# showlab/VideoSwap

Hardware: NVIDIA H100
Metric: denoise-steps/sec, 16f 512^2 SD1.5 UNet3D (CFG UNet fwd + CFG combine + DDIM step) (higher is better)
Workload: dtype f16

## Files before the change

### include/videoswap_b200.h

```cpp
#ifndef VIDEOSWAP_B200_H
#define VIDEOSWAP_B200_H
#include <stddef.h>
#include <stdint.h>

#ifdef __cplusplus
extern "C" {
#endif

const char* vs_last_error(void);
int vs_version(void);

typedef struct vs_unet_config {
  int in_channels, out_channels;
  int block_out_channels[4];
  int layers_per_block;
  int num_heads;
  int cross_attention_dim;
  int norm_num_groups;
  float norm_eps;
  int use_motion_module;
  int motion_down[4];
  int motion_up[4];
  int motion_mid;
  int motion_num_heads;
  int pe_max_len;
} vs_unet_config;

typedef struct vs_unet vs_unet;

int vs_unet_create(const vs_unet_config* cfg, vs_unet** out);
void vs_unet_destroy(vs_unet* h);

int vs_unet_load_weights(vs_unet* h, void* stream, int n, const char* const* names, const void* const* d_ptrs,
                         const int64_t* numels);
int vs_unet_num_params(const vs_unet* h);
const char* vs_unet_param_name(const vs_unet* h, int i);

int vs_unet_forward(vs_unet* h, void* stream, const void* d_sample, int io_f32, int B, int F, int H, int W,
                    const float* d_timesteps, const void* d_ehs, int ehs_tokens, int ehs_layers,
                    const void* const* d_residuals, int residuals_nhwc, float residual_scale, void* d_out);
int vs_unet_forward_features(vs_unet* h, void* stream, const void* d_sample, int io_f32, int B, int F, int H, int W,
                             const float* d_timesteps, const void* d_ehs, int ehs_tokens, int ehs_layers, int up_ft_index,
                             void* d_feat);
int vs_unet_time_embedding(vs_unet* h, void* stream, const float* d_timesteps, int B, float* d_emb, float* d_proj);
size_t vs_unet_workspace_bytes(const vs_unet* h);
int vs_unet_pin_workspace(vs_unet* h, int pin);
int vs_unet_reserve_workspace(vs_unet* h, int B, int F, int H, int W);
typedef struct vs_comm vs_comm;
int vs_comm_unique_id(void* out128);
int vs_comm_create(const void* id128, int rank, int nranks, vs_comm** out);
void vs_comm_destroy(vs_comm* c);
int vs_comm_all_gather(vs_comm* c, void* stream, const void* d_send, void* d_recv, size_t bytes_per_rank);
int vs_comm_all_reduce_sum_f32(vs_comm* c, void* stream, float* d_buf, size_t n);
int vs_unet_set_frame_shard(vs_unet* h, vs_comm* frame_comm, int shard, int nshards);

typedef void (*vs_attention_hook)(void* user, int layer, int is_cross, int place, void* d_probs, int batch, int heads, int nq,
                                  int nk, void* stream);
int vs_unet_set_attention_hook(vs_unet* h, vs_attention_hook hook, void* user, int max_queries);
int vs_attention_probs(void* stream, const void* d_q, int ldq, const void* d_k, int ldk, void* d_probs, int batch, int nq, int nk,
                       int heads, int d, long long q_bstride, long long kv_bstride, int kv_div);
int vs_attention_apply_probs(void* stream, const void* d_probs, const void* d_v, int ldv, void* d_o, int ldo, int batch, int nq,
                             int nk, int heads, int d, long long kv_bstride, long long o_bstride, int kv_div);
int vs_blend_mask(void* stream, const void* const* d_maps, int n_maps, int n_prompts, int frames, int heads, int res_h, int res_w,
                  int words, const float* d_alpha, int pool, int h, int w, float threshold, int both, float* d_mask);
int vs_latent_blend(void* stream, const void* d_x_src, void* d_x_tgt, const float* d_mask, int io_f32, int channels, int frames,
                    int hw);

int vs_unet_enable_taps(vs_unet* h, int enable);
int vs_unet_num_taps(const vs_unet* h);
int vs_unet_get_tap(const vs_unet* h, int i, const char** name, const void** d_ptr, int* nimg, int* hh, int* ww, int* c);
int vs_unet_copy_tap(const vs_unet* h, void* stream, int i, void* d_dst);

int vs_cfg_ddim_step(void* stream, const void* d_eps2, const void* d_latents, int io_f32, size_t n, int cfg,
                     float guidance, float alpha_t, float alpha_prev, void* d_out);

int vs_cfg_ddim_step_dev(void* stream, const void* d_eps2, const void* d_latents, int io_f32, size_t n, int cfg,
                         float guidance, const float* d_coef, void* d_out);

int vs_cfg_ddim_rescale_step(void* stream, const void* d_eps2, const void* d_latents, const void* d_noise, int io_f32, int S,
                             size_t n_s, int cfg, float guidance, float alpha_t, float alpha_prev, float eta,
                             float guidance_rescale, void* d_out);

int vs_cfg_ddim_rescale_step_dev(void* stream, const void* d_eps2, const void* d_latents, const void* d_noise, int io_f32,
                                 int S, size_t n_s, int cfg, float guidance, const float* d_coef, void* d_out);

int vs_adapter_level(void* stream, const void* d_w0, const void* d_b0, const void* d_w1, const void* d_b1, int E, int mid,
                     int C, const float* d_point_embedding, const float* d_tracks, const int* d_point_mask, int F, int P,
                     int h, int w, float rate, int coord_fp16, float scale, float* d_ws, void* d_map);

typedef struct vs_gemm_desc {
  const void* A; int K1; int lda1;
  const void* A2; int K2; int lda2;
  const void* Bw;
  int M, N;
  int taps;
  int sub_py, sub_px;
  int nimg, H, W;
  const float* bias;
  const float* rowvec; int ldrv; int pix_per_batch; int rv_mod;
  const float* ln_stats; const float* ln_u;
  const float* ln_parts; int ln_nparts;
  float* ln_sums_out;
  const void* residual; int ldr;
  void* out; int ldc;
  int mode;
  int force_bn;
  int OH, OW;
  int stride2;
} vs_gemm_desc;
int vs_gemm_ex(void* stream, const vs_gemm_desc* desc);
int vs_pack_conv3x3(void* stream, const void* d_w, int cout, int cin, void* d_out);
int vs_pack_geglu(void* stream, const void* d_w, const void* d_b, int hidden, int K, void* d_wout, float* d_bout);
int vs_groupnorm(void* stream, const void* d_x1, int c1, const void* d_x2, int c2, int nimg, int hw, int imgs_per_set,
                 int groups, float eps, const float* d_gamma, const float* d_beta, int silu, float* d_sums, void* d_out);
int vs_groupnorm_stats(void* stream, const void* d_x1, int c1, const void* d_x2, int c2, int nimg, int hw, int imgs_per_set,
                       int groups, float* d_sums, int zero_first);
int vs_groupnorm_apply(void* stream, const void* d_x1, int c1, const void* d_x2, int c2, int nimg, int hw, int imgs_per_set,
                       int groups, const float* d_sums, float eps, const float* d_gamma, const float* d_beta, int silu,
                       int count_scale, void* d_out);
int vs_layernorm(void* stream, const void* d_x, int rows, int C, const float* d_gamma, const float* d_beta,
                 const float* d_pe, int hw, int F, void* d_out);
int vs_ln_linear(void* stream, const void* d_x, int M, int C, const void* d_w, const float* d_bias, int N,
                 const float* d_gamma, const float* d_beta, const float* d_pe, int pe_len, int hw, int frames, int mode,
                 void* d_wf, float* d_u, float* d_c, float* d_cpe, float* d_stats, void* d_out);
int vs_linear_ln_linear(void* stream, const void* d_x0, int M, int K0, const void* d_w0, const float* d_b0,
                        const void* d_residual, int C, void* d_x, const void* d_w, const float* d_bias, int N,
                        const float* d_gamma, const float* d_beta, const float* d_pe, int pe_len, int hw, int frames,
                        int mode, void* d_wf, float* d_u, float* d_c, float* d_cpe, float* d_parts, int parts_capacity,
                        void* d_out);
int vs_attention(void* stream, const void* d_q, int ldq, const void* d_k, int ldk, const void* d_v, int ldv, void* d_o,
                 int ldo, int batch, int nq, int nk, int heads, int d, long long q_bstride, long long kv_bstride,
                 long long o_bstride, int kv_div);
int vs_temporal_attention(void* stream, const void* d_qkv, void* d_o, int B, int F, int HW, int C, int heads);
int vs_conv_in(void* stream, const void* d_x, int nimg, int H, int W, int cin, const void* d_w, const float* d_bias,
               int cout, void* d_scratch, void* d_out);
int vs_upsample2x(void* stream, const void* d_x, int nimg, int H, int W, int C, void* d_out);
int vs_upsample_conv3x3(void* stream, const void* d_x, int nimg, int H, int W, int C, const void* d_w, int Cout,
                        const float* d_bias, void* d_wsub, void* d_out);
int vs_upsample_conv3x3_sized(void* stream, const void* d_x, int nimg, int H, int W, int C, const void* d_w, int Cout,
                              const float* d_bias, int OH, int OW, void* d_wpanels, void* d_out);
int vs_upsample_nearest(void* stream, const void* d_x, int nimg, int H, int W, int C, int OH, int OW, void* d_out);
int vs_conv3x3_s2(void* stream, const void* d_x, int nimg, int H, int W, int C, const void* d_w_packed, int Cout,
                  const float* d_bias, void* d_scratch, void* d_out);

int vs_pack_conv_subpixel(void* stream, const void* d_w, int cout, int cin, void* d_out);
int vs_softmax_rows(void* stream, void* d_s, int rows, int n, int ld, float scale);
int vs_transpose_pad(void* stream, const void* d_src, int rows, int cols, int rows_pad, void* d_dst);
int vs_vae_latent_in(void* stream, const void* d_z, int z_is_f32, int nimg, int h, int w, float divisor, const float* d_wb,
                     void* d_out);
int vs_image_postprocess(void* stream, const void* d_x, int nimg, int H, int W, int channels, int format, void* d_out);

int vs_downsample_conv3x3(void* stream, const void* d_x, int nimg, int H, int W, int C, const void* d_w_packed, int Cout,
                          const float* d_bias, void* d_out);
int vs_vae_image_in(void* stream, const void* d_x, int src_format, int nimg, int H, int W, void* d_out);
int vs_vae_moments(void* stream, const void* d_x, int nimg, int h, int w, const float* d_wb, void* d_out);
int vs_vae_posterior(void* stream, const void* d_params, const void* d_noise, int nimg, int h, int w, float scale, int layout,
                     void* d_out);

int vs_clip_embed(void* stream, const int* d_ids_i32, int n, int L, const void* d_tok, int vocab, const void* d_pos, int C,
                  void* d_out);
int vs_causal_attention(void* stream, const void* d_qkv, int ldqkv, void* d_o, int ldo, int nseq, int L, int heads, int d);

int vs_dift_noise(void* stream, const void* d_moments, const float* d_eps1, const float* d_eps2, int n, int E, int h, int w,
                  float sf, float sqrt_a, float sqrt_1ma, float* d_out);
int vs_dift_point_sample(void* stream, const void* d_feat, int n, int E, int h, int w, int C, int H, int W, const int* d_xy,
                         int P, float* d_out);
int vs_dift_ensemble_mean(void* stream, const void* d_feat, int n, int E, int h, int w, int C, float* d_out);
int vs_dift_point_reduce(void* stream, const float* d_vecs, int n, int P, int C, const float* d_src, const int* d_src_row,
                         float* d_conf, const void* d_accept, float* d_sums, float* d_counts, float* d_means);

typedef struct vs_imlp_desc {
  const float* d_params;
  int input_dim;
  int output_dim;
  int hidden_dim;
  int mlp_layers;
  int pe_dim;
  uint32_t skip_mask;
  int use_tanh;
} vs_imlp_desc;
int vs_imlp_forward(void* stream, const vs_imlp_desc* net, const float* d_x, int rows, float* d_out);
int vs_atlas_propagate(void* stream, const vs_imlp_desc* fg, const vs_imlp_desc* fg_inverse, const vs_imlp_desc* alpha,
                       const float* d_points, float t_key, int P, int F, int larger_dim, float* d_ws, float* d_tracks);

int vs_profile_enable(int on);
int vs_profile_reset(void);
int vs_profile_collect(int category, double* ms, double* work, long long* count);
long long vs_launch_count(void);
int vs_profile_dump(const char* path);
int vs_set_option(const char* name, int value);

#ifdef __cplusplus
}
#endif
#endif
```

### videoswap_b200/_lib.py

```python
from __future__ import annotations

import ctypes as C
import os
import re

HERE = os.path.dirname(os.path.abspath(__file__))
LIB_PATH = os.path.join(HERE, "libvideoswap_b200.so")
HEADER_PATH = os.path.join(os.path.dirname(HERE), "include", "videoswap_b200.h")


class VSError(RuntimeError):
    pass


class UNetConfigStruct(C.Structure):
    _fields_ = [
        ("in_channels", C.c_int), ("out_channels", C.c_int), ("block_out_channels", C.c_int * 4),
        ("layers_per_block", C.c_int), ("num_heads", C.c_int), ("cross_attention_dim", C.c_int),
        ("norm_num_groups", C.c_int), ("norm_eps", C.c_float), ("use_motion_module", C.c_int),
        ("motion_down", C.c_int * 4), ("motion_up", C.c_int * 4), ("motion_mid", C.c_int),
        ("motion_num_heads", C.c_int), ("pe_max_len", C.c_int),
    ]


_P = C.c_void_p
_I = C.c_int
_F = C.c_float
_LL = C.c_longlong
_SZ = C.c_size_t


class ImlpDescStruct(C.Structure):
    _fields_ = [("params", _P), ("input_dim", _I), ("output_dim", _I), ("hidden_dim", _I), ("mlp_layers", _I),
                ("pe_dim", _I), ("skip_mask", C.c_uint32), ("use_tanh", _I)]


class GemmDescStruct(C.Structure):
    _fields_ = [
        ("A", _P), ("K1", _I), ("lda1", _I),
        ("A2", _P), ("K2", _I), ("lda2", _I),
        ("Bw", _P),
        ("M", _I), ("N", _I),
        ("taps", _I),
        ("sub_py", _I), ("sub_px", _I),
        ("nimg", _I), ("H", _I), ("W", _I),
        ("bias", _P),
        ("rowvec", _P), ("ldrv", _I), ("pix_per_batch", _I), ("rv_mod", _I),
        ("ln_stats", _P), ("ln_u", _P),
        ("ln_parts", _P), ("ln_nparts", _I),
        ("ln_sums_out", _P),
        ("residual", _P), ("ldr", _I),
        ("out", _P), ("ldc", _I),
        ("mode", _I),
        ("force_bn", _I),
        ("OH", _I), ("OW", _I),
        ("stride2", _I),
    ]

_SIGNATURES = {
    "vs_last_error": (C.c_char_p, []),
    "vs_version": (_I, []),
    "vs_unet_create": (_I, [C.POINTER(UNetConfigStruct), C.POINTER(_P)]),
    "vs_unet_destroy": (None, [_P]),
    "vs_unet_load_weights": (_I, [_P, _P, _I, C.POINTER(C.c_char_p), C.POINTER(_P), C.POINTER(C.c_int64)]),
    "vs_unet_num_params": (_I, [_P]),
    "vs_unet_param_name": (C.c_char_p, [_P, _I]),
    "vs_unet_forward": (_I, [_P, _P, _P, _I, _I, _I, _I, _I, _P, _P, _I, _I, C.POINTER(_P), _I, _F, _P]),
    "vs_unet_time_embedding": (_I, [_P, _P, _P, _I, _P, _P]),
    "vs_unet_workspace_bytes": (_SZ, [_P]),
    "vs_unet_pin_workspace": (_I, [_P, _I]),
    "vs_unet_reserve_workspace": (_I, [_P, _I, _I, _I, _I]),
    "vs_comm_unique_id": (_I, [_P]),
    "vs_comm_create": (_I, [_P, _I, _I, C.POINTER(_P)]),
    "vs_comm_destroy": (None, [_P]),
    "vs_comm_all_gather": (_I, [_P, _P, _P, _P, _SZ]),
    "vs_comm_all_reduce_sum_f32": (_I, [_P, _P, _P, _SZ]),
    "vs_unet_set_frame_shard": (_I, [_P, _P, _I, _I]),
    "vs_unet_enable_taps": (_I, [_P, _I]),
    "vs_unet_num_taps": (_I, [_P]),
    "vs_unet_get_tap": (_I, [_P, _I, C.POINTER(C.c_char_p), C.POINTER(_P), C.POINTER(_I), C.POINTER(_I), C.POINTER(_I),
                             C.POINTER(_I)]),
    "vs_unet_copy_tap": (_I, [_P, _P, _I, _P]),
    "vs_profile_enable": (_I, [_I]),
    "vs_profile_reset": (_I, []),
    "vs_profile_collect": (_I, [_I, C.POINTER(C.c_double), C.POINTER(C.c_double), C.POINTER(C.c_longlong)]),
    "vs_launch_count": (C.c_longlong, []),
    "vs_set_option": (_I, [C.c_char_p, _I]),
    "vs_profile_dump": (_I, [C.c_char_p]),
    "vs_cfg_ddim_step": (_I, [_P, _P, _P, _I, _SZ, _I, _F, _F, _F, _P]),
    "vs_cfg_ddim_step_dev": (_I, [_P, _P, _P, _I, _SZ, _I, _F, _P, _P]),
    "vs_cfg_ddim_rescale_step": (_I, [_P, _P, _P, _P, _I, _I, _SZ, _I, _F, _F, _F, _F, _F, _P]),
    "vs_cfg_ddim_rescale_step_dev": (_I, [_P, _P, _P, _P, _I, _I, _SZ, _I, _F, _P, _P]),
    "vs_adapter_level": (_I, [_P, _P, _P, _P, _P, _I, _I, _I, _P, _P, _P, _I, _I, _I, _I, _F, _I, _F, _P, _P]),
    "vs_gemm_ex": (_I, [_P, C.POINTER(GemmDescStruct)]),
    "vs_pack_conv3x3": (_I, [_P, _P, _I, _I, _P]),
    "vs_pack_geglu": (_I, [_P, _P, _P, _I, _I, _P, _P]),
    "vs_groupnorm": (_I, [_P, _P, _I, _P, _I, _I, _I, _I, _I, _F, _P, _P, _I, _P, _P]),
    "vs_groupnorm_stats": (_I, [_P, _P, _I, _P, _I, _I, _I, _I, _I, _P, _I]),
    "vs_groupnorm_apply": (_I, [_P, _P, _I, _P, _I, _I, _I, _I, _I, _P, _F, _P, _P, _I, _I, _P]),
    "vs_layernorm": (_I, [_P, _P, _I, _I, _P, _P, _P, _I, _I, _P]),
    "vs_ln_linear": (_I, [_P, _P, _I, _I, _P, _P, _I, _P, _P, _P, _I, _I, _I, _I, _P, _P, _P, _P, _P, _P]),
    "vs_unet_set_attention_hook": (_I, [_P, _P, _P, _I]),
    "vs_attention_probs": (_I, [_P, _P, _I, _P, _I, _P, _I, _I, _I, _I, _I, _LL, _LL, _I]),
    "vs_attention_apply_probs": (_I, [_P, _P, _P, _I, _P, _I, _I, _I, _I, _I, _I, _LL, _LL, _I]),
    "vs_blend_mask": (_I, [_P, _P, _I, _I, _I, _I, _I, _I, _I, _P, _I, _I, _I, _F, _I, _P]),
    "vs_latent_blend": (_I, [_P, _P, _P, _P, _I, _I, _I, _I]),
    "vs_linear_ln_linear": (_I, [_P, _P, _I, _I, _P, _P, _P, _I, _P, _P, _P, _I, _P, _P, _P, _I, _I, _I, _I, _P, _P, _P, _P,
                                 _P, _I, _P]),
    "vs_attention": (_I, [_P, _P, _I, _P, _I, _P, _I, _P, _I, _I, _I, _I, _I, _I, _LL, _LL, _LL, _I]),
    "vs_temporal_attention": (_I, [_P, _P, _P, _I, _I, _I, _I, _I]),
    "vs_conv_in": (_I, [_P, _P, _I, _I, _I, _I, _P, _P, _I, _P, _P]),
    "vs_upsample2x": (_I, [_P, _P, _I, _I, _I, _I, _P]),
    "vs_upsample_conv3x3": (_I, [_P, _P, _I, _I, _I, _I, _P, _I, _P, _P, _P]),
    "vs_upsample_conv3x3_sized": (_I, [_P, _P, _I, _I, _I, _I, _P, _I, _P, _I, _I, _P, _P]),
    "vs_upsample_nearest": (_I, [_P, _P, _I, _I, _I, _I, _I, _I, _P]),
    "vs_conv3x3_s2": (_I, [_P, _P, _I, _I, _I, _I, _P, _I, _P, _P, _P]),
    "vs_pack_conv_subpixel": (_I, [_P, _P, _I, _I, _P]),
    "vs_softmax_rows": (_I, [_P, _P, _I, _I, _I, _F]),
    "vs_transpose_pad": (_I, [_P, _P, _I, _I, _I, _P]),
    "vs_vae_latent_in": (_I, [_P, _P, _I, _I, _I, _I, _F, _P, _P]),
    "vs_image_postprocess": (_I, [_P, _P, _I, _I, _I, _I, _I, _P]),
    "vs_downsample_conv3x3": (_I, [_P, _P, _I, _I, _I, _I, _P, _I, _P, _P]),
    "vs_vae_image_in": (_I, [_P, _P, _I, _I, _I, _I, _P]),
    "vs_vae_moments": (_I, [_P, _P, _I, _I, _I, _P, _P]),
    "vs_vae_posterior": (_I, [_P, _P, _P, _I, _I, _I, _F, _I, _P]),
    "vs_clip_embed": (_I, [_P, _P, _I, _I, _P, _I, _P, _I, _P]),
    "vs_causal_attention": (_I, [_P, _P, _I, _P, _I, _I, _I, _I, _I]),
    "vs_unet_forward_features": (_I, [_P, _P, _P, _I, _I, _I, _I, _I, _P, _P, _I, _I, _I, _P]),
    "vs_dift_noise": (_I, [_P, _P, _P, _P, _I, _I, _I, _I, _F, _F, _F, _P]),
    "vs_dift_point_sample": (_I, [_P, _P, _I, _I, _I, _I, _I, _I, _I, _P, _I, _P]),
    "vs_dift_ensemble_mean": (_I, [_P, _P, _I, _I, _I, _I, _I, _P]),
    "vs_dift_point_reduce": (_I, [_P, _P, _I, _I, _I, _P, _P, _P, _P, _P, _P, _P]),
    "vs_imlp_forward": (_I, [_P, C.POINTER(ImlpDescStruct), _P, _I, _P]),
    "vs_atlas_propagate": (_I, [_P, C.POINTER(ImlpDescStruct), C.POINTER(ImlpDescStruct), C.POINTER(ImlpDescStruct), _P, _F,
                                _I, _I, _I, _P, _P]),
}

_lib = None


def header_symbols():
    with open(HEADER_PATH) as f:
        text = f.read()
    text = re.sub(r"/\*.*?\*/", "", text, flags=re.S)
    return sorted(set(re.findall(r"\b(vs_[a-z0-9_]+)\s*\(", text)))


def lib() -> C.CDLL:
    global _lib
    if _lib is None:
        if not os.path.exists(LIB_PATH):
            raise VSError(f"{LIB_PATH} is missing: build it with `python -m videoswap_b200.build` "
                          f"(there is no CPU/PyTorch fallback for this path)")
        _lib = C.CDLL(LIB_PATH)
        for name, (res, args) in _SIGNATURES.items():
            fn = getattr(_lib, name)
            fn.restype = res
            fn.argtypes = args
    return _lib


def check(code: int, what: str = ""):
    if code != 0:
        msg = lib().vs_last_error()
        raise VSError(f"{what or 'videoswap_b200 call'} failed ({code}): {msg.decode() if msg else '?'}")


def call(name: str, *args):
    check(getattr(lib(), name)(*args), name)
```

### videoswap_b200/csrc/api.cu

```cuda
#include "../../include/videoswap_b200.h"
#include "common.cuh"
#include "kernels.h"

using namespace vs;

extern "C" const char* vs_last_error(void) { return vs::last_error(); }
extern "C" int vs_version(void) { return 100; }

extern "C" int vs_cfg_ddim_step(void* stream, const void* d_eps2, const void* d_latents, int io_f32, size_t n, int cfg,
                                float guidance, float alpha_t, float alpha_prev, void* d_out) {
  VS_REQUIRE(d_eps2 && d_latents && d_out, "vs_cfg_ddim_step: null pointer");
  VS_REQUIRE(alpha_t > 0.f && alpha_t <= 1.f && alpha_prev > 0.f && alpha_prev <= 1.f, "vs_cfg_ddim_step: alphas must be in (0,1]");
  return cfg_ddim_step((cudaStream_t)stream, d_eps2, d_latents, io_f32, n, cfg, guidance, alpha_t, alpha_prev, d_out);
}

extern "C" int vs_cfg_ddim_step_dev(void* stream, const void* d_eps2, const void* d_latents, int io_f32, size_t n, int cfg,
                                    float guidance, const float* d_coef, void* d_out) {
  VS_REQUIRE(d_eps2 && d_latents && d_out && d_coef, "vs_cfg_ddim_step_dev: null pointer");
  return cfg_ddim_step_dev((cudaStream_t)stream, d_eps2, d_latents, io_f32, n, cfg, guidance, d_coef, d_out);
}

extern "C" int vs_cfg_ddim_rescale_step(void* stream, const void* d_eps2, const void* d_latents, const void* d_noise,
                                        int io_f32, int S, size_t n_s, int cfg, float guidance, float alpha_t,
                                        float alpha_prev, float eta, float guidance_rescale, void* d_out) {
  VS_REQUIRE(d_eps2 && d_latents && d_out && (d_noise || eta == 0.f), "vs_cfg_ddim_rescale_step: null pointer");
  VS_REQUIRE(S > 0 && n_s > 0, "vs_cfg_ddim_rescale_step: S = %d and n_s = %zu must be > 0", S, n_s);
  VS_REQUIRE(alpha_t > 0.f && alpha_t <= 1.f && alpha_prev > 0.f && alpha_prev <= 1.f,
             "vs_cfg_ddim_rescale_step: alphas must be in (0,1]");
  VS_REQUIRE(eta >= 0.f && (eta == 0.f || alpha_t < 1.f), "vs_cfg_ddim_rescale_step: eta must be >= 0 (and alpha_t < 1 when > 0)");
  VS_REQUIRE(guidance_rescale >= 0.f, "vs_cfg_ddim_rescale_step: guidance_rescale must be >= 0");
  return cfg_ddim_rescale_step((cudaStream_t)stream, d_eps2, d_latents, d_noise, io_f32, S, n_s, cfg, guidance, alpha_t,
                               alpha_prev, eta, guidance_rescale, d_out);
}

extern "C" int vs_cfg_ddim_rescale_step_dev(void* stream, const void* d_eps2, const void* d_latents, const void* d_noise,
                                            int io_f32, int S, size_t n_s, int cfg, float guidance, const float* d_coef,
                                            void* d_out) {
  VS_REQUIRE(d_eps2 && d_latents && d_out && d_coef, "vs_cfg_ddim_rescale_step_dev: null pointer");
  VS_REQUIRE(S > 0 && n_s > 0, "vs_cfg_ddim_rescale_step_dev: S = %d and n_s = %zu must be > 0", S, n_s);
  return cfg_ddim_rescale_step_dev((cudaStream_t)stream, d_eps2, d_latents, d_noise, io_f32, S, n_s, cfg, guidance, d_coef,
                                   d_out);
}

extern "C" int vs_adapter_level(void* stream, const void* d_w0, const void* d_b0, const void* d_w1, const void* d_b1, int E,
                                int mid, int C, const float* d_pe, const float* d_tracks, const int* d_mask, int F, int P,
                                int h, int w, float rate, int coord_fp16, float scale, float* d_ws, void* d_map) {
  cudaStream_t st = (cudaStream_t)stream;
  VS_REQUIRE(d_w0 && d_b0 && d_w1 && d_b1 && d_pe && d_tracks && d_ws && d_map, "vs_adapter_level: null pointer");
  float* b0 = d_ws;
  float* b1 = b0 + mid;
  float* hid = b1 + C;
  float* feat = hid + (size_t)P * mid;
  if (int e = f16_to_f32(st, (const __half*)d_b0, mid, b0)) return e;
  if (int e = f16_to_f32(st, (const __half*)d_b1, C, b1)) return e;
  if (int e = small_linear(st, d_pe, P, E, (const __half*)d_w0, b0, mid, false, true, hid)) return e;
  if (int e = small_linear(st, hid, P, mid, (const __half*)d_w1, b1, C, false, false, feat)) return e;
  return adapter_splat(st, feat, d_tracks, d_mask, F, P, C, h, w, rate, coord_fp16, scale, (__half*)d_map);
}

extern "C" int vs_gemm_ex(void* stream, const vs_gemm_desc* d) {
  VS_REQUIRE(d != nullptr, "vs_gemm_ex: null descriptor");
  GemmArgs g;
  g.A = (const __half*)d->A; g.K1 = d->K1; g.lda1 = d->lda1;
  g.A2 = (const __half*)d->A2; g.K2 = d->K2; g.lda2 = d->lda2;
  g.Bw = (const __half*)d->Bw;
  g.M = d->M; g.N = d->N;
  g.taps = d->taps;
  g.sub_py = d->sub_py; g.sub_px = d->sub_px;
  g.nimg = d->nimg; g.H = d->H; g.W = d->W;
  g.bias = d->bias;
  g.rowvec = d->rowvec; g.ldrv = d->ldrv; g.pix_per_batch = d->pix_per_batch; g.rv_mod = d->rv_mod;
  g.ln_stats = d->ln_stats; g.ln_u = d->ln_u;
  g.ln_parts = d->ln_parts; g.ln_nparts = d->ln_nparts;
  g.ln_sums_out = d->ln_sums_out;
  g.residual = (const __half*)d->residual; g.ldr = d->ldr;
  g.out = (__half*)d->out; g.ldc = d->ldc;
  g.mode = d->mode;
  g.force_bn = d->force_bn;
  g.OH = d->OH; g.OW = d->OW;
  g.stride2 = d->stride2;
  return gemm_tc((cudaStream_t)stream, g);
}

extern "C" int vs_pack_conv3x3(void* stream, const void* d_w, int cout, int cin, void* d_out) {
  return pack_conv3x3((cudaStream_t)stream, (const __half*)d_w, cout, cin, (__half*)d_out);
}
extern "C" int vs_pack_geglu(void* stream, const void* d_w, const void* d_b, int hidden, int K, void* d_wout, float* d_bout) {
  cudaStream_t st = (cudaStream_t)stream;
  if (int e = pack_geglu(st, (const __half*)d_w, nullptr, hidden, K, kGegluGranule, (__half*)d_wout, nullptr)) return e;
  return pack_geglu(st, nullptr, (const __half*)d_b, hidden, 1, kGegluGranule, nullptr, d_bout);
}

extern "C" int vs_groupnorm(void* stream, const void* d_x1, int c1, const void* d_x2, int c2, int nimg, int hw,
                            int imgs_per_set, int groups, float eps, const float* d_gamma, const float* d_beta, int silu,
                            float* d_sums, void* d_out) {
  cudaStream_t st = (cudaStream_t)stream;
  if (imgs_per_set == 1 && c2 == 0) {
    const int e = groupnorm_frame_fused(st, (const __half*)d_x1, c1, nimg, hw, groups, eps, d_gamma, d_beta, silu != 0, (__half*)d_out);
    if (e >= 0) return e;
  }
  if (int e = groupnorm_stats(st, (const __half*)d_x1, c1, (const __half*)d_x2, c2, nimg, hw, imgs_per_set, groups, d_sums)) return e;
  return groupnorm_apply(st, (const __half*)d_x1, c1, (const __half*)d_x2, c2, nimg, hw, imgs_per_set, groups, d_sums, eps,
                         d_gamma, d_beta, silu != 0, (__half*)d_out);
}
extern "C" int vs_groupnorm_stats(void* stream, const void* d_x1, int c1, const void* d_x2, int c2, int nimg, int hw,
                                  int imgs_per_set, int groups, float* d_sums, int zero_first) {
  VS_REQUIRE(d_sums != nullptr, "vs_groupnorm_stats: null sums");
  return groupnorm_stats((cudaStream_t)stream, (const __half*)d_x1, c1, (const __half*)d_x2, c2, nimg, hw, imgs_per_set, groups,
                         d_sums, zero_first != 0);
}
extern "C" int vs_groupnorm_apply(void* stream, const void* d_x1, int c1, const void* d_x2, int c2, int nimg, int hw,
                                  int imgs_per_set, int groups, const float* d_sums, float eps, const float* d_gamma,
                                  const float* d_beta, int silu, int count_scale, void* d_out) {
  VS_REQUIRE(d_sums && d_out, "vs_groupnorm_apply: null pointer");
  VS_REQUIRE(count_scale >= 1, "vs_groupnorm_apply: count_scale must be >= 1");
  return groupnorm_apply((cudaStream_t)stream, (const __half*)d_x1, c1, (const __half*)d_x2, c2, nimg, hw, imgs_per_set, groups,
                         d_sums, eps, d_gamma, d_beta, silu != 0, (__half*)d_out, count_scale);
}
extern "C" int vs_layernorm(void* stream, const void* d_x, int rows, int C, const float* d_gamma, const float* d_beta,
                            const float* d_pe, int hw, int F, void* d_out) {
  return layernorm((cudaStream_t)stream, (const __half*)d_x, rows, C, d_gamma, d_beta, d_pe, hw, F, (__half*)d_out);
}
extern "C" int vs_ln_linear(void* stream, const void* d_x, int M, int C, const void* d_w, const float* d_bias, int N,
                            const float* d_gamma, const float* d_beta, const float* d_pe, int pe_len, int hw, int frames,
                            int mode, void* d_wf, float* d_u, float* d_c, float* d_cpe, float* d_stats, void* d_out) {
  cudaStream_t st = (cudaStream_t)stream;
  if (int e = ln_fold(st, (const __half*)d_w, N, C, d_gamma, d_beta, d_bias, d_pe, pe_len, (__half*)d_wf, d_u, d_c, d_cpe)) return e;
  if (int e = ln_rowstats(st, (const __half*)d_x, M, C, d_stats)) return e;
  GemmArgs g;
  g.A = (const __half*)d_x; g.K1 = C; g.lda1 = C; g.Bw = (const __half*)d_wf; g.M = M; g.N = N; g.bias = d_c;
  g.ln_stats = d_stats; g.ln_u = d_u; g.out = (__half*)d_out; g.ldc = mode == EPI_GEGLU ? N / 2 : N; g.mode = mode;
  if (d_pe) { g.rowvec = d_cpe; g.ldrv = N; g.pix_per_batch = hw; g.rv_mod = frames; }
  return gemm_tc(st, g);
}
extern "C" int vs_upsample_conv3x3(void* stream, const void* d_x, int nimg, int H, int W, int C, const void* d_w, int Cout,
                                   const float* d_bias, void* d_wsub, void* d_out) {
  cudaStream_t st = (cudaStream_t)stream;
  if (int e = pack_conv_subpixel(st, (const __half*)d_w, Cout, C, (__half*)d_wsub)) return e;
  for (int par = 0; par < 4; ++par) {
    GemmArgs g;
    g.A = (const __half*)d_x; g.K1 = C; g.lda1 = C; g.Bw = (const __half*)d_wsub + (size_t)par * Cout * 4 * C; g.taps = 4;
    g.sub_py = par >> 1; g.sub_px = par & 1; g.nimg = nimg; g.H = H; g.W = W; g.M = nimg * H * W; g.N = Cout; g.bias = d_bias;
    g.out = (__half*)d_out; g.ldc = Cout;
    if (int e = gemm_tc(st, g)) return e;
  }
  return 0;
}
extern "C" int vs_upsample_conv3x3_sized(void* stream, const void* d_x, int nimg, int H, int W, int C, const void* d_w, int Cout,
                                         const float* d_bias, int OH, int OW, void* d_wpanels, void* d_out) {
  cudaStream_t st = (cudaStream_t)stream;
  VS_REQUIRE(d_x && d_w && d_wpanels && d_out && nimg >= 1 && H >= 1 && W >= 1, "vs_upsample_conv3x3_sized: bad arguments");
  __half* w3x3 = (__half*)d_wpanels;
  __half* wsub = w3x3 + (size_t)Cout * 9 * C;
  if (int e = pack_conv3x3(st, (const __half*)d_w, Cout, C, w3x3)) return e;
  if (int e = pack_conv_subpixel(st, (const __half*)d_w, Cout, C, wsub, true)) return e;
  return upsample_conv3x3(st, (const __half*)d_x, nimg, H, W, C, w3x3, wsub, d_bias, Cout, OH, OW, (__half*)d_out);
}
extern "C" int vs_upsample_nearest(void* stream, const void* d_x, int nimg, int H, int W, int C, int OH, int OW, void* d_out) {
  return upsample_nearest2x((cudaStream_t)stream, (const __half*)d_x, nimg, H, W, C, (__half*)d_out, OH, OW);
}
extern "C" int vs_attention_probs(void* stream, const void* d_q, int ldq, const void* d_k, int ldk, void* d_probs, int batch, int nq,
                                  int nk, int heads, int d, long long q_bstride, long long kv_bstride, int kv_div) {
  return attention_probs((cudaStream_t)stream, (const __half*)d_q, ldq, (const __half*)d_k, ldk, (__half*)d_probs, batch, nq, nk, heads,
                         d, q_bstride, kv_bstride, kv_div);
}
extern "C" int vs_attention_apply_probs(void* stream, const void* d_probs, const void* d_v, int ldv, void* d_o, int ldo, int batch,
                                        int nq, int nk, int heads, int d, long long kv_bstride, long long o_bstride, int kv_div) {
  return attention_apply_probs((cudaStream_t)stream, (const __half*)d_probs, (const __half*)d_v, ldv, (__half*)d_o, ldo, batch, nq, nk,
                               heads, d, kv_bstride, o_bstride, kv_div);
}
extern "C" int vs_blend_mask(void* stream, const void* const* d_maps, int n_maps, int n_prompts, int frames, int heads, int res_h,
                             int res_w, int words, const float* d_alpha, int pool, int h, int w, float threshold, int both,
                             float* d_mask) {
  const int res[2] = {res_h, res_w};
  return blend_mask((cudaStream_t)stream, (const __half* const*)d_maps, res, n_maps, n_prompts, frames, heads, words, d_alpha, pool, h, w,
                    threshold, both, d_mask);
}
extern "C" int vs_latent_blend(void* stream, const void* d_x_src, void* d_x_tgt, const float* d_mask, int io_f32, int channels,
                               int frames, int hw) {
  return latent_blend((cudaStream_t)stream, d_x_src, d_x_tgt, d_mask, io_f32, channels, frames, hw);
}
extern "C" int vs_linear_ln_linear(void* stream, const void* d_x0, int M, int K0, const void* d_w0, const float* d_b0,
                                   const void* d_residual, int C, void* d_x, const void* d_w, const float* d_bias, int N,
                                   const float* d_gamma, const float* d_beta, const float* d_pe, int pe_len, int hw,
                                   int frames, int mode, void* d_wf, float* d_u, float* d_c, float* d_cpe, float* d_parts,
                                   int parts_capacity, void* d_out) {
  cudaStream_t st = (cudaStream_t)stream;
  if (int e = ln_fold(st, (const __half*)d_w, N, C, d_gamma, d_beta, d_bias, d_pe, pe_len, (__half*)d_wf, d_u, d_c, d_cpe)) return e;
  GemmArgs g0;
  g0.A = (const __half*)d_x0; g0.K1 = K0; g0.lda1 = K0; g0.Bw = (const __half*)d_w0; g0.M = M; g0.N = C; g0.bias = d_b0;
  g0.residual = (const __half*)d_residual; g0.ldr = C; g0.out = (__half*)d_x; g0.ldc = C; g0.ln_sums_out = d_parts;
  const int parts = gemm_n_tiles(g0);
  VS_REQUIRE(parts >= 1 && parts <= parts_capacity, "vs_linear_ln_linear: %d partial-sum slices do not fit the buffer (%d)", parts, parts_capacity);
  if (int e = gemm_tc(st, g0)) return e;
  GemmArgs g;
  g.A = (const __half*)d_x; g.K1 = C; g.lda1 = C; g.Bw = (const __half*)d_wf; g.M = M; g.N = N; g.bias = d_c;
  g.ln_parts = d_parts; g.ln_nparts = parts; g.ln_u = d_u; g.out = (__half*)d_out; g.ldc = mode == EPI_GEGLU ? N / 2 : N; g.mode = mode;
  if (d_pe) { g.rowvec = d_cpe; g.ldrv = N; g.pix_per_batch = hw; g.rv_mod = frames; }
  return gemm_tc(st, g);
}
extern "C" int vs_attention(void* stream, const void* d_q, int ldq, const void* d_k, int ldk, const void* d_v, int ldv,
                            void* d_o, int ldo, int batch, int nq, int nk, int heads, int d, long long q_bstride,
                            long long kv_bstride, long long o_bstride, int kv_div) {
  return attention((cudaStream_t)stream, (const __half*)d_q, ldq, (const __half*)d_k, ldk, (const __half*)d_v, ldv,
                   (__half*)d_o, ldo, batch, nq, nk, heads, d, q_bstride, kv_bstride, o_bstride, kv_div);
}
extern "C" int vs_temporal_attention(void* stream, const void* d_qkv, void* d_o, int B, int F, int HW, int C, int heads) {
  return temporal_attention((cudaStream_t)stream, (const __half*)d_qkv, (__half*)d_o, B, F, HW, C, heads);
}
extern "C" int vs_conv_in(void* stream, const void* d_x, int nimg, int H, int W, int cin, const void* d_w, const float* d_bias,
                          int cout, void* d_scratch, void* d_out) {
  return conv_in_3x3((cudaStream_t)stream, (const __half*)d_x, nimg, H, W, cin, (const __half*)d_w, d_bias, cout, (__half*)d_out,
                     (__half*)d_scratch);
}
extern "C" int vs_upsample2x(void* stream, const void* d_x, int nimg, int H, int W, int C, void* d_out) {
  return upsample_nearest2x((cudaStream_t)stream, (const __half*)d_x, nimg, H, W, C, (__half*)d_out);
}
extern "C" int vs_conv3x3_s2(void* stream, const void* d_x, int nimg, int H, int W, int C, const void* d_w, int Cout,
                             const float* d_bias, void* d_scratch, void* d_out) {
  cudaStream_t st = (cudaStream_t)stream;
  if (int e = im2col_s2(st, (const __half*)d_x, nimg, H, W, C, (__half*)d_scratch)) return e;
  const int Ho = (H - 1) / 2 + 1, Wo = (W - 1) / 2 + 1;
  GemmArgs g;
  g.A = (const __half*)d_scratch; g.K1 = 9 * C; g.lda1 = 9 * C; g.Bw = (const __half*)d_w; g.M = nimg * Ho * Wo; g.N = Cout;
  g.bias = d_bias; g.out = (__half*)d_out; g.ldc = Cout;
  return gemm_tc(st, g);
}

extern "C" int vs_pack_conv_subpixel(void* stream, const void* d_w, int cout, int cin, void* d_out) {
  VS_REQUIRE(d_w && d_out, "vs_pack_conv_subpixel: null pointer");
  return pack_conv_subpixel((cudaStream_t)stream, (const __half*)d_w, cout, cin, (__half*)d_out);
}
extern "C" int vs_softmax_rows(void* stream, void* d_s, int rows, int n, int ld, float scale) {
  return softmax_rows((cudaStream_t)stream, (__half*)d_s, rows, n, ld, scale);
}
extern "C" int vs_transpose_pad(void* stream, const void* d_src, int rows, int cols, int rows_pad, void* d_dst) {
  return transpose_pad((cudaStream_t)stream, (const __half*)d_src, rows, cols, rows_pad, (__half*)d_dst);
}
extern "C" int vs_vae_latent_in(void* stream, const void* d_z, int z_is_f32, int nimg, int h, int w, float divisor,
                                const float* d_wb, void* d_out) {
  return vae_latent_in((cudaStream_t)stream, d_z, z_is_f32, nimg, h, w, divisor, d_wb, (__half*)d_out);
}
extern "C" int vs_image_postprocess(void* stream, const void* d_x, int nimg, int H, int W, int channels, int format, void* d_out) {
  return image_postprocess((cudaStream_t)stream, (const __half*)d_x, nimg, H, W, channels, format, d_out);
}
extern "C" int vs_downsample_conv3x3(void* stream, const void* d_x, int nimg, int H, int W, int C, const void* d_w_packed,
                                     int Cout, const float* d_bias, void* d_out) {
  VS_REQUIRE(d_x && d_w_packed && d_out, "vs_downsample_conv3x3: null pointer");
  GemmArgs g;
  g.A = (const __half*)d_x; g.K1 = C; g.lda1 = C; g.Bw = (const __half*)d_w_packed; g.taps = 9; g.stride2 = 1;
  g.nimg = nimg; g.H = H; g.W = W; g.M = nimg * (H / 2) * (W / 2); g.N = Cout; g.bias = d_bias; g.out = (__half*)d_out;
  g.ldc = Cout;
  return gemm_tc((cudaStream_t)stream, g);
}
extern "C" int vs_vae_image_in(void* stream, const void* d_x, int src_format, int nimg, int H, int W, void* d_out) {
  return vae_image_in((cudaStream_t)stream, d_x, src_format, nimg, H, W, (__half*)d_out);
}
extern "C" int vs_vae_moments(void* stream, const void* d_x, int nimg, int h, int w, const float* d_wb, void* d_out) {
  return vae_moments((cudaStream_t)stream, (const __half*)d_x, nimg, h, w, d_wb, (__half*)d_out);
}
extern "C" int vs_vae_posterior(void* stream, const void* d_params, const void* d_noise, int nimg, int h, int w, float scale,
                                int layout, void* d_out) {
  return vae_posterior((cudaStream_t)stream, (const __half*)d_params, (const __half*)d_noise, nimg, h, w, scale, layout,
                       (__half*)d_out);
}
extern "C" int vs_clip_embed(void* stream, const int* d_ids_i32, int n, int L, const void* d_tok, int vocab, const void* d_pos, int C,
                             void* d_out) {
  return clip_embed((cudaStream_t)stream, d_ids_i32, n, L, (const __half*)d_tok, vocab, (const __half*)d_pos, C, (__half*)d_out);
}
extern "C" int vs_causal_attention(void* stream, const void* d_qkv, int ldqkv, void* d_o, int ldo, int nseq, int L, int heads,
                                   int d) {
  return causal_attention((cudaStream_t)stream, (const __half*)d_qkv, ldqkv, (__half*)d_o, ldo, nseq, L, heads, d);
}

extern "C" int vs_dift_noise(void* stream, const void* d_moments, const float* d_eps1, const float* d_eps2, int n, int E, int h,
                             int w, float sf, float sqrt_a, float sqrt_1ma, float* d_out) {
  return dift_noise((cudaStream_t)stream, (const __half*)d_moments, d_eps1, d_eps2, n, E, h, w, sf, sqrt_a, sqrt_1ma, d_out);
}
extern "C" int vs_dift_point_sample(void* stream, const void* d_feat, int n, int E, int h, int w, int C, int H, int W,
                                    const int* d_xy, int P, float* d_out) {
  return dift_point_sample((cudaStream_t)stream, (const __half*)d_feat, n, E, h, w, C, H, W, d_xy, P, d_out);
}
extern "C" int vs_dift_ensemble_mean(void* stream, const void* d_feat, int n, int E, int h, int w, int C, float* d_out) {
  return dift_ensemble_mean((cudaStream_t)stream, (const __half*)d_feat, n, E, h, w, C, d_out);
}
extern "C" int vs_dift_point_reduce(void* stream, const float* d_vecs, int n, int P, int C, const float* d_src,
                                    const int* d_src_row, float* d_conf, const void* d_accept, float* d_sums, float* d_counts,
                                    float* d_means) {
  return dift_point_reduce((cudaStream_t)stream, d_vecs, n, P, C, d_src, d_src_row, d_conf, (const uint8_t*)d_accept, d_sums,
                           d_counts, d_means);
}

extern "C" int vs_profile_enable(int on) { prof_enable(on != 0); return 0; }
extern "C" int vs_profile_reset(void) { prof_reset(); return 0; }
extern "C" int vs_profile_collect(int category, double* ms, double* work, long long* count) {
  VS_REQUIRE(category >= 0 && category < PC_COUNT && ms && work && count, "vs_profile_collect: bad argument");
  return prof_collect(category, ms, work, count);
}
extern "C" long long vs_launch_count(void) { return launch_count(); }
extern "C" int vs_profile_dump(const char* path) {
  VS_REQUIRE(path != nullptr, "vs_profile_dump: null path");
  return prof_dump(path);
}
extern "C" int vs_set_option(const char* name, int value) {
  VS_REQUIRE(name != nullptr, "vs_set_option: null name");
  return set_option(name, value);
}
```

### videoswap_b200/csrc/gemm.cu

```cuda
#include <type_traits>

#include "common.cuh"
#include "kernels.h"

namespace vs {

namespace {

constexpr int BM = 128;
constexpr int WG_M = 64;
constexpr int BK = 64;
constexpr int A_STAGE_BYTES = BM * BK * 2;
constexpr uint64_t A_HALF_DESC = (WG_M * BK * 2) >> 4;
constexpr int GEMM_THREADS = 384;
constexpr int SMEM_LIMIT = 227 * 1024;
constexpr int EPI_COLS = 32;
constexpr int EPI_WARP_BYTES = 16 * 64;
constexpr int EPI_BYTES = 8 * EPI_WARP_BYTES;
constexpr int PRODUCER_REGS = 40, CONSUMER_REGS = 232;
enum { EPI_F_GEGLU = 1, EPI_F_RES = 2, EPI_F_RV = 4, EPI_F_LN = 8, EPI_F_LNOUT = 16, EPI_F_QGELU = 32 };

struct GemmParams {
  CUtensorMap tmA, tmA2, tmB;
  int M, N;
  int num_kb;
  int kb_per_tap;
  int kb_src1;
  int taps;
  int a_rank;
  int nimg, H, W, TH, TW, TN, tiles_x, tiles_y;
  int tap_x0, tap_y0, tap_w;
  int osy, osx, ooy, oox, OH, OW;
  int tw_log, thw_log;
  int m_tiles, n_tiles;
  const float* bias;
  const float* rowvec;
  int ldrv;
  int pix_per_batch;
  int rv_mod;
  const float2* ln_stats;
  const float* ln_u;
  const float2* ln_parts;
  int ln_nparts;
  float ln_inv_c;
  float2* ln_sums_out;
  const __half* residual;
  int ldr;
  __half* out;
  int ldc;
  int staged;
  int stages;
};

struct GemmParamsSub : GemmParams {
  CUtensorMap tmS[3];
  int sub_short;
};

struct GemmParamsS2 : GemmParams {
  CUtensorMap tmP[3];
};

constexpr int LN_MAX_PARTS = 8;
struct GemmParamsEpi : GemmParams {
  CUtensorMap tmR;
};

template <int BN, int EPI>
struct EpiSlot {
  static constexpr bool RES = (EPI & EPI_F_RES) != 0, LN = (EPI & EPI_F_LN) != 0, RV = (EPI & EPI_F_RV) != 0;
  static constexpr int RES_BYTES = RES ? BM * BN * 2 : 0;
  static constexpr int BIAS_OFF = RES_BYTES;
  static constexpr int U_OFF = BIAS_OFF + BN * 4;
  static constexpr int RV_OFF = U_OFF + (LN ? BN * 4 : 0);
  static constexpr int LNR_OFF = RV_OFF + (RV ? 2 * BN * 4 : 0);
  static constexpr int END = LNR_OFF + (LN ? LN_MAX_PARTS * BM * 8 : 0);
  static constexpr int BYTES = RES ? (END + 1023) / 1024 * 1024 : (END + 127) / 128 * 128;
};

template <int BN, int SLOT_BYTES = 0>
struct Cfg {
  static constexpr bool COOP = BN > 160;
  static constexpr int HALVES = COOP ? 1 : 2;
  static constexpr int B_STAGE_BYTES = BN * BK * 2;
  static constexpr int STAGE_BYTES = A_STAGE_BYTES + B_STAGE_BYTES;
  static constexpr int STAGES_RAW = SLOT_BYTES ? (SMEM_LIMIT - 1024 - 256 - EPI_BYTES - 2 * SLOT_BYTES) / STAGE_BYTES
                                               : (SMEM_LIMIT - 2048 - EPI_BYTES) / STAGE_BYTES;
  static constexpr int STAGES = STAGES_RAW > 12 ? 12 : STAGES_RAW;
  static constexpr int SMEM_BYTES =
      STAGES * STAGE_BYTES + EPI_BYTES + 2 * SLOT_BYTES + 1024  + 256 ;
  static_assert(B_STAGE_BYTES % 1024 == 0, "B stage must keep 1024-byte alignment for SWIZZLE_128B");
  static_assert(STAGES >= 3, "pipeline too shallow");
  static_assert(SMEM_BYTES <= SMEM_LIMIT, "shared memory");
  static_assert(BN % 32 == 0 && BN <= 256, "wgmma N");
};

__device__ __forceinline__ uint32_t sw64_off(int row, int chunk) {
  return (uint32_t)(row * 64 + ((chunk ^ ((row >> 1) & 3)) << 4));
}

template <int BN, int EPI, typename Params>
__global__ void __launch_bounds__(GEMM_THREADS, 1) gemm_tc_kernel(const __grid_constant__ Params p) {
  constexpr bool SUB = std::is_same<Params, GemmParamsSub>::value;
  constexpr bool S2 = std::is_same<Params, GemmParamsS2>::value;
  constexpr bool SLOT = std::is_same<Params, GemmParamsEpi>::value;
  using ES = EpiSlot<BN, EPI>;
  using C = Cfg<BN, SLOT ? ES::BYTES : 0>;
  static_assert(!SLOT || ((C::COOP == ((EPI & EPI_F_GEGLU) != 0)) && (EPI & EPI_F_QGELU) == 0), "epilogue slots: ping-pong linears and cooperative GEGLUs");
  constexpr bool GEGLU = (EPI & EPI_F_GEGLU) != 0, HAS_RES = (EPI & EPI_F_RES) != 0, HAS_RV = (EPI & EPI_F_RV) != 0;
  constexpr bool LN = (EPI & EPI_F_LN) != 0;
  constexpr bool LNOUT = (EPI & EPI_F_LNOUT) != 0;
  constexpr bool QGELU = (EPI & EPI_F_QGELU) != 0;
  extern __shared__ uint8_t smem_raw[];
  const uint32_t smem_base = (smem_u32(smem_raw) + 1023u) & ~1023u;
  const uint32_t epi_base = smem_base + C::STAGES * C::STAGE_BYTES;
  const uint32_t slot_base = epi_base + EPI_BYTES;
  const uint32_t bar_base = slot_base + (SLOT ? 2 * ES::BYTES : 0);
  auto full_bar = [&](int s) { return bar_base + 8u * s; };
  auto empty_bar = [&](int s) { return bar_base + 8u * (C::STAGES + s); };
  auto slot_full = [&](int g) { return bar_base + 8u * (2 * C::STAGES + g); };
  auto slot_empty = [&](int g) { return bar_base + 8u * (2 * C::STAGES + 2 + g); };

  const int warp = threadIdx.x >> 5;
  const int lane = threadIdx.x & 31;
  const int wg = threadIdx.x >> 7;
  const int nst = (p.stages > 0 && p.stages < C::STAGES) ? p.stages : C::STAGES;
  const int total_tiles = p.m_tiles * p.n_tiles;

  if (threadIdx.x == 0) {
    prefetch_tmap(&p.tmA);
    prefetch_tmap(&p.tmB);
    if (p.kb_src1 < p.kb_per_tap) prefetch_tmap(&p.tmA2);
    if constexpr (SUB) {
      if (p.sub_short & 1) prefetch_tmap(&p.tmS[0]);
      if (p.sub_short & 2) prefetch_tmap(&p.tmS[1]);
      if (p.sub_short == 3) prefetch_tmap(&p.tmS[2]);
    }
    if constexpr (S2) {
      for (int k = 0; k < 3; ++k) prefetch_tmap(&p.tmP[k]);
    }
    if constexpr (SLOT) {
      if (ES::RES) prefetch_tmap(&p.tmR);
      for (int g = 0; g < 2; ++g) {
        mbar_init(slot_full(g), 1);
        mbar_init(slot_empty(g), C::COOP ? 8 : 4);
      }
    }
    for (int s = 0; s < C::STAGES; ++s) {
      mbar_init(full_bar(s), 1);
      mbar_init(empty_bar(s), C::COOP ? 8 : 4);
    }
    fence_barrier_init();
  }
  __syncthreads();
  pdl_trigger();
  pdl_wait();

  if (wg == 0) {
    setmaxnreg_dec<PRODUCER_REGS>();
    if constexpr (SLOT) {
      if (warp == 1) {
        for (int t = blockIdx.x, j = 0; t < total_tiles; t += gridDim.x, ++j) {
          const int g = j & 1;
          mbar_wait(slot_empty(g), ((j >> 1) & 1) ^ 1);
          if (elect_one()) {
            const int m_tile = t / p.n_tiles, n_tile = t % p.n_tiles;
            const int n0 = n_tile * BN, m0 = m_tile * BM;
            const int ncols = p.N - n0 < BN ? p.N - n0 : BN;
            const int parts = p.ln_nparts > 0 ? p.ln_nparts : 1;
            const int rows = p.M - m0 < BM ? p.M - m0 : BM;
            const int last = m0 + rows - 1;
            int rv0 = m0 / p.pix_per_batch, rv1 = last / p.pix_per_batch;
            const int nrv = rv1 != rv0 ? 2 : 1;
            if (p.rv_mod > 0) { rv0 %= p.rv_mod; rv1 %= p.rv_mod; }
            const uint32_t sb = slot_base + (uint32_t)g * ES::BYTES, fb = slot_full(g);
            uint32_t bytes = p.bias != nullptr ? ncols * 4u : 0u;
            if (ES::RES) bytes += (uint32_t)(ncols / EPI_COLS) * (BM * 64);
            if (ES::LN) bytes += ncols * 4u + (uint32_t)(parts * rows) * 8u;
            if (ES::RV) bytes += (uint32_t)nrv * ncols * 4u;
            mbar_expect_tx(fb, bytes);
            if (p.bias != nullptr) bulk_load(sb + ES::BIAS_OFF, p.bias + n0, ncols * 4u, fb);
            if constexpr (ES::RES) {
              for (int c = 0; c < ncols / EPI_COLS; ++c) tma_load_2d(sb + c * (BM * 64), &p.tmR, fb, n0 + c * EPI_COLS, m0);
            }
            if constexpr (ES::LN) {
              bulk_load(sb + ES::U_OFF, p.ln_u + n0, ncols * 4u, fb);
              const float2* src = p.ln_nparts > 0 ? p.ln_parts : p.ln_stats;
              for (int k = 0; k < parts; ++k)
                bulk_load(sb + ES::LNR_OFF + k * (BM * 8), src + (long long)k * p.M + m0, rows * 8u, fb);
            }
            if constexpr (ES::RV) {
              bulk_load(sb + ES::RV_OFF, p.rowvec + (long long)rv0 * p.ldrv + n0, ncols * 4u, fb);
              if (nrv == 2) bulk_load(sb + ES::RV_OFF + BN * 4, p.rowvec + (long long)rv1 * p.ldrv + n0, ncols * 4u, fb);
            }
          }
          __syncwarp();
        }
        return;
      }
    }
    if (warp != 0) return;
    const int num_kb = p.num_kb, kb_per_tap = p.kb_per_tap, kb_src1 = p.kb_src1;
    const bool conv = p.a_rank == 4;
    const int tap_x0 = p.tap_x0, tap_x1 = p.tap_x0 + p.tap_w;
    bool short_y = false, short_x = false;
    if constexpr (SUB) { short_y = (p.sub_short & 1) != 0; short_x = (p.sub_short & 2) != 0; }
    uint32_t pr_s = 0, pr_ph = 0;
    for (int t = blockIdx.x; t < total_tiles; t += gridDim.x) {
      const int m_tile = t / p.n_tiles, n_tile = t % p.n_tiles;
      int x0 = 0, y0 = 0, i0 = 0;
      if (conv) {
        x0 = (m_tile % p.tiles_x) * p.TW;
        y0 = ((m_tile / p.tiles_x) % p.tiles_y) * p.TH;
        i0 = (m_tile / (p.tiles_x * p.tiles_y)) * p.TN;
      }
      const int n0 = n_tile * BN;
      const int m0 = m_tile * BM;
      int kcoord = 0;
      int dy = p.tap_y0, dx = tap_x0;
      int r = 0;
      for (int kb = 0; kb < num_kb; ++kb) {
        mbar_wait(empty_bar(pr_s), pr_ph ^ 1);
        if (elect_one()) {
          const uint32_t fb = full_bar(pr_s);
          const uint32_t a_dst = smem_base + pr_s * C::STAGE_BYTES;
          const bool first = r < kb_src1;
          const CUtensorMap* tm = first ? &p.tmA : &p.tmA2;
          if constexpr (SUB) {
            const bool sy = short_y && dy == p.tap_y0 + 2, sx = short_x && dx == tap_x0 + 2;
            if (sy || sx) tm = sy ? (sx ? &p.tmS[2] : &p.tmS[0]) : &p.tmS[1];
          }
          int ox = dx, oy = dy;
          if constexpr (S2) {
            const int par = ((dy & 1) << 1) | (dx & 1);
            if (par) tm = &p.tmP[par - 1];
            ox = dx >> 1; oy = dy >> 1;
          }
          const int c = (first ? r : r - kb_src1) * BK;
          mbar_expect_tx(fb, C::STAGE_BYTES);
          if (conv) tma_load_4d(a_dst, tm, fb, c, x0 + ox, y0 + oy, i0);
          else tma_load_2d(a_dst, tm, fb, c, m0);
          tma_load_2d(a_dst + A_STAGE_BYTES, &p.tmB, fb, kcoord, n0);
        }
        __syncwarp();
        kcoord += BK;
        if (++r == kb_per_tap) {
          r = 0;
          if (++dx == tap_x1) { dx = tap_x0; ++dy; }
        }
        if (++pr_s == (uint32_t)nst) { pr_s = 0; pr_ph ^= 1; }
      }
    }
    return;
  }

  setmaxnreg_inc<CONSUMER_REGS>();
  const int g = wg - 1;
  const int wq = warp & 3;
  const int q = lane & 3;
  const int rbase = 16 * wq + (lane >> 2);
  const uint32_t stage_buf = epi_base + (uint32_t)(warp - 4) * EPI_WARP_BYTES;
  const bool has_bias = p.bias != nullptr;
  const bool staged = SLOT || p.staged != 0;
  const int num_kb = p.num_kb;
  auto tile_pixel = [&](int m_tile, int row) -> int {
    if (p.a_rank == 4) {
      const int x0 = (m_tile % p.tiles_x) * p.TW;
      const int y0 = ((m_tile / p.tiles_x) % p.tiles_y) * p.TH;
      const int i0 = (m_tile / (p.tiles_x * p.tiles_y)) * p.TN;
      const int ti = row >> p.thw_log, rem = row & ((1 << p.thw_log) - 1);
      const int y = y0 + (rem >> p.tw_log), x = x0 + (rem & (p.TW - 1)), img = i0 + ti;
      if constexpr (SUB) {
        const int oy = y * p.osy + p.ooy, ox = x * p.osx + p.oox;
        return ((img < p.nimg) && (y < p.H) && (x < p.W) && (oy < p.OH) && (ox < p.OW)) ? (img * p.OH + oy) * p.OW + ox : -1;
      }
      return ((img < p.nimg) && (y < p.H) && (x < p.W)) ? (img * p.OH + y * p.osy + p.ooy) * p.OW + x * p.osx + p.oox : -1;
    }
    const int px = m_tile * BM + row;
    return px < p.M ? px : -1;
  };

  const int bar_mine = 1 + g, bar_other = 2 - g;
  float acc[C::HALVES][BN / 2];
  uint32_t s = 0, ph = 0;
  for (int t = blockIdx.x, j = 0; t < total_tiles; t += gridDim.x, ++j) {
    const int m_tile = t / p.n_tiles, n_tile = t % p.n_tiles;
    if (!C::COOP && (j & 1) != g) {
      const uint32_t sn = s + (uint32_t)num_kb;
      ph ^= (sn / (uint32_t)nst) & 1u;
      s = sn % (uint32_t)nst;
      continue;
    }
    if (!C::COOP && j > 0) named_bar_sync(bar_mine, 256);
    uint32_t prev = 0;
    for (int kb = 0; kb < num_kb; ++kb) {
      mbar_wait(full_bar(s), ph);
      wgmma_fence();
      const uint32_t a_addr = smem_base + s * C::STAGE_BYTES;
      const uint64_t da = gmma_desc_sw128(a_addr) + (C::COOP ? (uint64_t)g * A_HALF_DESC : 0);
      const uint64_t db = gmma_desc_sw128(a_addr + A_STAGE_BYTES);
#pragma unroll
      for (int k = 0; k < BK / 16; ++k) {
#pragma unroll
        for (int hh = 0; hh < C::HALVES; ++hh)
          wgmma_ss<BN>(acc[hh], da + hh * A_HALF_DESC + 2 * k, db + 2 * k, (kb | k) != 0 ? 1u : 0u);
      }
      wgmma_commit();
      if (kb > 0) {
        wgmma_wait<1>();
        if (lane == 0) mbar_arrive(empty_bar(prev));
      }
      prev = s;
      if (++s == (uint32_t)nst) { s = 0; ph ^= 1; }
    }
    if (!C::COOP && t + (int)gridDim.x < total_tiles) named_bar_arrive(bar_other, 256);
    wgmma_wait<0>();
    if (lane == 0) mbar_arrive(empty_bar(prev));
    const int js = j & 1;
    const uint8_t* slot = smem_raw + (slot_base + (uint32_t)js * ES::BYTES - smem_u32(smem_raw));
    if constexpr (SLOT) mbar_wait(slot_full(js), (uint32_t)(j >> 1) & 1u);

    const int n0 = n_tile * BN;
#pragma unroll
    for (int hh = 0; hh < C::HALVES; ++hh) {
      const int r0 = WG_M * (C::COOP ? g : hh) + rbase;
      int pix[2];
      pix[0] = tile_pixel(m_tile, r0);
      pix[1] = tile_pixel(m_tile, r0 + 8);
      const float* rv[2] = {nullptr, nullptr};
      if (SLOT && HAS_RV) {
#pragma unroll
        for (int h = 0; h < 2; ++h) {
          const int d = pix[h] >= 0 ? pix[h] / p.pix_per_batch - (m_tile * BM) / p.pix_per_batch : 0;
          rv[h] = reinterpret_cast<const float*>(slot + ES::RV_OFF) + d * BN;
        }
      } else if (HAS_RV || !staged) {
#pragma unroll
        for (int h = 0; h < 2; ++h) {
          if (p.rowvec != nullptr && pix[h] >= 0) {
            int ri = pix[h] / p.pix_per_batch;
            if (p.rv_mod > 0) ri %= p.rv_mod;
            rv[h] = p.rowvec + (long long)ri * p.ldrv + n0;
          }
        }
      }
      if (staged) {
        constexpr int OC = GEGLU ? BN / 2 : BN;
        const int oc0 = n_tile * OC;
        const int nsub = (p.N - n0 < BN ? (GEGLU ? (p.N - n0) / 2 : p.N - n0) : OC) / EPI_COLS;
        float la[2] = {1.f, 1.f}, lb[2] = {0.f, 0.f};
        if (LN) {
#pragma unroll
          for (int h = 0; h < 2; ++h) {
            if (pix[h] < 0) continue;
            const float2* lnr = reinterpret_cast<const float2*>(slot + ES::LNR_OFF) + r0 + 8 * h;
            if (p.ln_nparts > 0) {
              float S = 0.f, Q = 0.f;
              for (int k = 0; k < p.ln_nparts; ++k) {
                const float2 v = SLOT ? lnr[k * BM] : __ldg(p.ln_parts + (long long)k * p.M + pix[h]);
                S += v.x; Q += v.y;
              }
              const float mean = S * p.ln_inv_c;
              la[h] = rsqrtf(fmaxf(fmaf(-mean, mean, Q * p.ln_inv_c), 0.f) + 1e-5f);
              lb[h] = -mean * la[h];
            } else {
              const float2 st2 = SLOT ? lnr[0] : __ldg(p.ln_stats + pix[h]);
              la[h] = st2.x; lb[h] = st2.y;
            }
          }
        }
        float rs[2] = {0.f, 0.f}, rq[2] = {0.f, 0.f};
        __half* orow[2];
        const __half* rrow[2];
#pragma unroll
        for (int h = 0; h < 2; ++h) {
          const long long px = pix[h] >= 0 ? pix[h] : 0;
          orow[h] = p.out + px * p.ldc + oc0 + q * 8;
          rrow[h] = HAS_RES ? p.residual + px * p.ldr + oc0 + q * 8 : nullptr;
        }
#pragma unroll
        for (int sb = 0; sb < OC / EPI_COLS; ++sb) {
          if (sb >= nsub) break;
          uint4 rr[2];
          if (SLOT && HAS_RES) {
#pragma unroll
            for (int h = 0; h < 2; ++h)
              rr[h] = *reinterpret_cast<const uint4*>(slot + sb * (BM * 64) + sw64_off(r0 + 8 * h, q));
          } else if (HAS_RES) {
#pragma unroll
            for (int h = 0; h < 2; ++h) rr[h] = __ldg(reinterpret_cast<const uint4*>(rrow[h] + sb * EPI_COLS));
          }
#pragma unroll
          for (int jj = 0; jj < 4; ++jj) {
            const int j = 4 * sb + jj;
            const int c = 8 * j + 2 * q;
            float2 b = make_float2(0.f, 0.f), u = make_float2(0.f, 0.f);
            if constexpr (SLOT) {
              if (has_bias) b = *reinterpret_cast<const float2*>(slot + ES::BIAS_OFF + 4 * c);
              if (LN) u = *reinterpret_cast<const float2*>(slot + ES::U_OFF + 4 * c);
            } else {
              if (has_bias) b = __ldg(reinterpret_cast<const float2*>(p.bias + n0 + c));
              if (LN) u = __ldg(reinterpret_cast<const float2*>(p.ln_u + n0 + c));
            }
            float2 bg = make_float2(0.f, 0.f), ug = make_float2(0.f, 0.f);
            if (GEGLU) {
              if constexpr (SLOT) {
                bg = *reinterpret_cast<const float2*>(slot + ES::BIAS_OFF + 4 * (BN / 2 + c));
                if (LN) ug = *reinterpret_cast<const float2*>(slot + ES::U_OFF + 4 * (BN / 2 + c));
              } else {
                bg = __ldg(reinterpret_cast<const float2*>(p.bias + n0 + BN / 2 + c));
                if (LN) ug = __ldg(reinterpret_cast<const float2*>(p.ln_u + n0 + BN / 2 + c));
              }
            }
#pragma unroll
            for (int h = 0; h < 2; ++h) {
              float f0 = acc[hh][4 * j + 2 * h], f1 = acc[hh][4 * j + 2 * h + 1];
              if (GEGLU) {
                float g0 = acc[hh][4 * (j + BN / 16) + 2 * h], g1 = acc[hh][4 * (j + BN / 16) + 2 * h + 1];
                float bv0 = b.x, bv1 = b.y, bg0 = bg.x, bg1 = bg.y;
                if (LN) {
                  bv0 = fmaf(lb[h], u.x, bv0); bv1 = fmaf(lb[h], u.y, bv1);
                  bg0 = fmaf(lb[h], ug.x, bg0); bg1 = fmaf(lb[h], ug.y, bg1);
                  f0 *= la[h]; f1 *= la[h]; g0 *= la[h]; g1 *= la[h];
                }
                f0 = (f0 + bv0) * gelu_sig(g0 + bg0);
                f1 = (f1 + bv1) * gelu_sig(g1 + bg1);
              } else {
                if (LN) {
                  f0 = fmaf(la[h], f0, fmaf(lb[h], u.x, b.x));
                  f1 = fmaf(la[h], f1, fmaf(lb[h], u.y, b.y));
                } else if (has_bias) {
                  f0 += b.x; f1 += b.y;
                }
                if (HAS_RV && rv[h] != nullptr) {
                  const float2 r2 = SLOT ? *reinterpret_cast<const float2*>(rv[h] + c)
                                         : __ldg(reinterpret_cast<const float2*>(rv[h] + c));
                  f0 += r2.x; f1 += r2.y;
                }
                if constexpr (QGELU) {
                  f0 = quick_gelu_f(f0); f1 = quick_gelu_f(f1);
                }
              }
              const __half2 hv = __floats2half2_rn(f0, f1);
              const uint32_t sa = stage_buf + sw64_off((lane >> 2) + 8 * h, jj) + 4 * q;
              if constexpr (SLOT)
                asm volatile("st.shared.b32 [%0], %1;" ::"r"(sa), "r"(*reinterpret_cast<const uint32_t*>(&hv)));
              else
                asm volatile("st.shared.b32 [%0], %1;" ::"r"(sa), "r"(*reinterpret_cast<const uint32_t*>(&hv)) : "memory");
            }
          }
          __syncwarp();
#pragma unroll
          for (int h = 0; h < 2; ++h) {
            uint4 o;
            asm volatile("ld.shared.v4.b32 {%0,%1,%2,%3}, [%4];" : "=r"(o.x), "=r"(o.y), "=r"(o.z), "=r"(o.w)
                         : "r"(stage_buf + sw64_off((lane >> 2) + 8 * h, q)));
            if (HAS_RES) {
              __half2* oh = reinterpret_cast<__half2*>(&o);
              const __half2* rh = reinterpret_cast<const __half2*>(&rr[h]);
#pragma unroll
              for (int t = 0; t < 4; ++t) oh[t] = __hadd2(oh[t], rh[t]);
            }
            if (pix[h] >= 0) *reinterpret_cast<uint4*>(orow[h] + sb * EPI_COLS) = o;
            if (LNOUT) {
              const __half2* oh = reinterpret_cast<const __half2*>(&o);
              const float2 a = __half22float2(oh[0]), b2 = __half22float2(oh[1]), c2 = __half22float2(oh[2]), d2 = __half22float2(oh[3]);
              rs[h] += ((a.x + a.y) + (b2.x + b2.y)) + ((c2.x + c2.y) + (d2.x + d2.y));
              float q0 = fmaf(a.x, a.x, a.y * a.y), q1 = fmaf(b2.x, b2.x, b2.y * b2.y);
              float q2 = fmaf(c2.x, c2.x, c2.y * c2.y), q3 = fmaf(d2.x, d2.x, d2.y * d2.y);
              rq[h] += (q0 + q1) + (q2 + q3);
            }
          }
          __syncwarp();
        }
        if (LNOUT) {
#pragma unroll
          for (int h = 0; h < 2; ++h) {
            rs[h] += __shfl_xor_sync(0xffffffffu, rs[h], 1); rq[h] += __shfl_xor_sync(0xffffffffu, rq[h], 1);
            rs[h] += __shfl_xor_sync(0xffffffffu, rs[h], 2); rq[h] += __shfl_xor_sync(0xffffffffu, rq[h], 2);
            if (q == 0 && pix[h] >= 0) p.ln_sums_out[(long long)n_tile * p.M + pix[h]] = make_float2(rs[h], rq[h]);
          }
        }
      } else {
#pragma unroll
        for (int j = 0; j < BN / 8; ++j) {
#pragma unroll
          for (int e = 0; e < 4; ++e) {
            const int h = e >> 1, c = 8 * j + 2 * q + (e & 1), n = n0 + c;
            if (n < p.N && pix[h] >= 0) {
              float f = acc[hh][4 * j + e];
              if (has_bias) f += p.bias[n];
              if (rv[h]) f += rv[h][c];
              __half y = __float2half_rn(f);
              if (p.residual) y = __hadd(y, p.residual[(long long)pix[h] * p.ldr + n]);
              p.out[(long long)pix[h] * p.ldc + n] = y;
            }
          }
        }
      }
    }
    if constexpr (SLOT) {
      __syncwarp();
      if (lane == 0) mbar_arrive(slot_empty(js));
    }
  }
}

struct ConvTile { int tw, th, tn; };

ConvTile pick_conv_tile(int nimg, int H, int W) {
  ConvTile best{1, 1, BM};
  long long best_cost = -1;
  for (int tw = 1; tw <= BM; tw *= 2) {
    for (int th = 1; tw * th <= BM; th *= 2) {
      const int tn = BM / (tw * th);
      if (tw > 256 || th > 256 || tn > 256) continue;
      const long long cost = (long long)((W + tw - 1) / tw) * tw * ((H + th - 1) / th) * th * ((nimg + tn - 1) / tn) * tn;
      if (best_cost < 0 || cost < best_cost || (cost == best_cost && tw > best.tw)) {
        best_cost = cost;
        best = ConvTile{tw, th, tn};
      }
    }
  }
  return best;
}

template <int BN, int EPI, typename Params = GemmParams>
int launch(cudaStream_t st, const Params& p) {
  using C = Cfg<BN, std::is_same<Params, GemmParamsEpi>::value ? EpiSlot<BN, EPI>::BYTES : 0>;
  static bool configured = false;
  if (!configured) {
    VS_CHECK_CUDA(cudaFuncSetAttribute(gemm_tc_kernel<BN, EPI, Params>, cudaFuncAttributeMaxDynamicSharedMemorySize, C::SMEM_BYTES));
    configured = true;
  }
  const int total = p.m_tiles * p.n_tiles;
  int ctas = num_sms();
  const int cap = get_option("gemm_ctas");
  if (cap > 0 && cap < ctas) ctas = cap;
  return launch_pdl(gemm_tc_kernel<BN, EPI, Params>, dim3(total < ctas ? total : ctas), dim3(GEMM_THREADS), C::SMEM_BYTES, st, 1, p);
}

template <int BN>
int launch_linear(cudaStream_t st, const GemmParams& p) {
  const int epi = (p.residual ? EPI_F_RES : 0) | (p.rowvec ? EPI_F_RV : 0) | ((p.ln_stats || p.ln_parts) ? EPI_F_LN : 0) |
                  (p.ln_sums_out ? EPI_F_LNOUT : 0);
  switch (epi) {
    case EPI_F_LNOUT: return launch<BN, EPI_F_LNOUT>(st, p);
    case EPI_F_LNOUT | EPI_F_RES: return launch<BN, EPI_F_LNOUT | EPI_F_RES>(st, p);
    case EPI_F_LN: return launch<BN, EPI_F_LN>(st, p);
    case EPI_F_LN | EPI_F_RV: return launch<BN, EPI_F_LN | EPI_F_RV>(st, p);
    case 0: return launch<BN, 0>(st, p);
    case EPI_F_RES: return launch<BN, EPI_F_RES>(st, p);
    case EPI_F_RV: return launch<BN, EPI_F_RV>(st, p);
    case EPI_F_RES | EPI_F_RV: return launch<BN, EPI_F_RES | EPI_F_RV>(st, p);
    default: set_error("gemm_tc: unsupported epilogue combination 0x%x", epi); return 2;
  }
}

template <int BN>
int launch_linear_slot(cudaStream_t st, const GemmParams& p, const GemmArgs& a) {
  const bool geglu = a.mode == EPI_GEGLU;
  if (get_option("gemm_epi_slot") == 0 || a.taps != 1 || (a.mode != EPI_LINEAR && !geglu) || !p.staged || p.num_kb > 10)
    return -1;
  const int epi = (p.residual ? EPI_F_RES : 0) | (p.rowvec ? EPI_F_RV : 0) | ((p.ln_stats || p.ln_parts) ? EPI_F_LN : 0) |
                  (p.ln_sums_out ? EPI_F_LNOUT : 0) | (geglu ? EPI_F_GEGLU : 0);
  if (geglu ? (BN != 256 || (epi & ~EPI_F_LN) != EPI_F_GEGLU)
            : (BN == 256 || (epi != EPI_F_RES && epi != EPI_F_LNOUT && epi != (EPI_F_LNOUT | EPI_F_RES) &&
                             epi != EPI_F_LN && epi != (EPI_F_LN | EPI_F_RV))))
    return -1;
  GemmParamsEpi pe;
  memset(&pe, 0, sizeof(pe));
  static_cast<GemmParams&>(pe) = p;
  if (p.rowvec && !(p.pix_per_batch >= BM || p.pix_per_batch == BM / 2)) return -1;
  if (epi & EPI_F_LN) {
    const void* rows = p.ln_parts ? static_cast<const void*>(p.ln_parts) : static_cast<const void*>(p.ln_stats);
    const int parts = p.ln_parts ? p.ln_nparts : 1;
    if (parts > LN_MAX_PARTS || (reinterpret_cast<uintptr_t>(rows) & 15) != 0 || (p.M & 1) != 0) return -1;
  }
  if (epi & EPI_F_RES) {
    const uint64_t dims[2] = {(uint64_t)p.N, (uint64_t)p.M};
    const uint64_t str[1] = {(uint64_t)p.ldr * 2};
    const uint32_t box[2] = {EPI_COLS, BM};
    if (make_tmap_f16(&pe.tmR, p.residual, 2, dims, str, box, 2)) return 3;
  }
  if constexpr (BN == 256) {
    return epi == EPI_F_GEGLU ? launch<BN, EPI_F_GEGLU>(st, pe) : launch<BN, EPI_F_GEGLU | EPI_F_LN>(st, pe);
  } else {
    switch (epi) {
      case EPI_F_RES: return launch<BN, EPI_F_RES>(st, pe);
      case EPI_F_LNOUT: return launch<BN, EPI_F_LNOUT>(st, pe);
      case EPI_F_LNOUT | EPI_F_RES: return launch<BN, EPI_F_LNOUT | EPI_F_RES>(st, pe);
      case EPI_F_LN: return launch<BN, EPI_F_LN>(st, pe);
      default: return launch<BN, EPI_F_LN | EPI_F_RV>(st, pe);
    }
  }
}

int pick_bn(int m_tiles, int N, int num_kb) {
  if (N <= 64) return 64;
  int best = 128;
  long long best_cost = -1;
  const int cand[3] = {128, 160, 256};
  for (int i = 0; i < 3; ++i) {
    const int bn = cand[i];
    if (bn != 128 && N % bn != 0) continue;
    const long long tiles = (long long)m_tiles * ((N + bn - 1) / bn);
    const long long waves = (tiles + num_sms() - 1) / num_sms();
    const long long cost = waves * (16 + bn / 8);
    if (best_cost < 0 || cost < best_cost || (cost == best_cost && num_kb >= 40)) {
      best_cost = cost;
      best = bn;
    }
  }
  return best;
}

int ilog2(int v) { int l = 0; while ((1 << l) < v) ++l; return l; }

}

int gemm_n_tiles(const GemmArgs& a) {
  if (a.taps != 1) return 0;
  int bn = a.force_bn;
  if (a.mode == EPI_GEGLU) bn = 2 * kGegluGranule;
  else if (bn == 0) bn = pick_bn((a.M + BM - 1) / BM, a.N, (a.K1 + BK - 1) / BK + a.K2 / BK);
  return (a.N + bn - 1) / bn;
}

int gemm_tc(cudaStream_t st, const GemmArgs& a) {
  VS_REQUIRE(a.A && a.Bw && a.out, "gemm_tc: null pointer");
  VS_REQUIRE(a.taps == 1 || a.taps == 9 || a.taps == 4, "gemm_tc: taps must be 1, 9 (3x3) or 4 (sub-pixel)");
  VS_REQUIRE(a.K1 % 8 == 0 && a.K2 % 8 == 0, "gemm_tc: K must be a multiple of 8 (TMA 16-byte strides)");
  VS_REQUIRE((long long)a.M * (a.ldc > a.ldr ? a.ldc : a.ldr) < (1LL << 40) && a.M < (1 << 30), "gemm_tc: M too large");
  const bool two = a.A2 != nullptr && a.K2 > 0;
  if (two || a.taps != 1) VS_REQUIRE(a.K1 % BK == 0 && a.K2 % BK == 0, "gemm_tc: concat/conv sources need C %% 64 == 0 (got %d,%d)", a.K1, a.K2);
  GemmParamsSub ps;
  memset(&ps, 0, sizeof(ps));
  GemmParams& p = ps;
  GemmParamsS2 p2;
  memset(&p2, 0, sizeof(p2));
  const bool sub = a.taps == 4;
  const int OH = sub && a.OH > 0 ? a.OH : 2 * a.H, OW = sub && a.OW > 0 ? a.OW : 2 * a.W;
  const int sub_ty = sub && a.sub_py == 0 && (OH & 1) ? 3 : 2, sub_tx = sub && a.sub_px == 0 && (OW & 1) ? 3 : 2;
  if (sub) VS_REQUIRE((OH == 2 * a.H || OH == 2 * a.H - 1) && (OW == 2 * a.W || OW == 2 * a.W - 1),
                      "gemm_tc: sub-pixel output %dx%d is not 2x (or 2x - 1) of the %dx%d input", OH, OW, a.H, a.W);
  const int ntaps = sub ? sub_ty * sub_tx : a.taps;
  const int Ktap = a.K1 + (two ? a.K2 : 0);
  const int Ktot = Ktap * ntaps;
  p.taps = ntaps;
  p.kb_src1 = (a.K1 + BK - 1) / BK;
  p.kb_per_tap = p.kb_src1 + (two ? a.K2 / BK : 0);
  p.num_kb = p.kb_per_tap * ntaps;
  p.M = a.M;
  p.N = a.N;
  p.bias = a.bias;
  p.rowvec = a.rowvec;
  p.ldrv = a.ldrv > 0 ? a.ldrv : a.N;
  p.pix_per_batch = a.pix_per_batch > 0 ? a.pix_per_batch : 1;
  p.rv_mod = a.rv_mod;
  p.ln_stats = reinterpret_cast<const float2*>(a.ln_stats);
  p.ln_u = a.ln_u;
  p.ln_parts = reinterpret_cast<const float2*>(a.ln_parts);
  p.ln_nparts = a.ln_parts ? a.ln_nparts : 0;
  p.ln_inv_c = 1.f / (float)(a.K1 + a.K2);
  p.ln_sums_out = reinterpret_cast<float2*>(a.ln_sums_out);
  if (a.ln_parts) VS_REQUIRE(a.ln_stats == nullptr && a.ln_nparts >= 1 && a.ln_nparts <= 16 && a.taps == 1, "gemm_tc: bad LayerNorm partial-sum input");
  if (a.ln_stats || a.ln_parts) VS_REQUIRE(a.ln_u != nullptr && a.bias != nullptr && a.residual == nullptr, "gemm_tc: folded LayerNorm needs u and c vectors and no residual");
  if (a.ln_sums_out) VS_REQUIRE(a.taps == 1 && a.mode == EPI_LINEAR && a.rowvec == nullptr && !a.ln_stats && !a.ln_parts,
                                "gemm_tc: row statistics output is implemented for plain linear layers (+ bias / residual)");
  p.residual = a.residual;
  p.ldr = a.ldr;
  p.out = a.out;
  p.ldc = a.ldc;
  p.stages = get_option("gemm_stages");

  const bool s2 = a.stride2 != 0;
  if (s2) VS_REQUIRE(a.taps == 9 && !two && a.H % 2 == 0 && a.W % 2 == 0 && a.lda1 == a.K1 && a.mode == EPI_LINEAR &&
                     !a.ln_stats && !a.ln_parts,
                     "gemm_tc: the stride-2 conv takes one dense NHWC source of even height and width (got %dx%d)", a.H, a.W);
  const int GH = s2 ? a.H / 2 : a.H, GW = s2 ? a.W / 2 : a.W;
  if (a.taps != 1) {
    VS_REQUIRE(a.nimg > 0 && GH > 0 && GW > 0 && a.M == a.nimg * GH * GW, "gemm_tc: bad conv geometry");
    p.a_rank = 4;
    if (s2) { p.tap_x0 = p.tap_y0 = 0; p.tap_w = 3; p.osy = p.osx = 1; p.ooy = p.oox = 0; p.OH = GH; p.OW = GW; }
    else if (a.taps == 9) { p.tap_x0 = p.tap_y0 = -1; p.tap_w = 3; p.osy = p.osx = 1; p.ooy = p.oox = 0; p.OH = a.H; p.OW = a.W; }
    else {
      VS_REQUIRE((a.sub_py | 1) == 1 && (a.sub_px | 1) == 1, "gemm_tc: sub-pixel parity must be 0 or 1");
      p.tap_y0 = a.sub_py - 1; p.tap_x0 = a.sub_px - 1; p.tap_w = sub_tx;
      ps.sub_short = (sub_ty == 3 ? 1 : 0) | (sub_tx == 3 ? 2 : 0);
      p.osy = p.osx = 2; p.ooy = a.sub_py; p.oox = a.sub_px; p.OH = OH; p.OW = OW;
    }
    const ConvTile t = pick_conv_tile(a.nimg, GH, GW);
    p.nimg = a.nimg; p.H = GH; p.W = GW; p.TW = t.tw; p.TH = t.th; p.TN = t.tn;
    p.tw_log = ilog2(t.tw);
    p.thw_log = ilog2(t.tw * t.th);
    p.tiles_x = (GW + t.tw - 1) / t.tw;
    p.tiles_y = (GH + t.th - 1) / t.th;
    p.m_tiles = p.tiles_x * p.tiles_y * ((a.nimg + t.tn - 1) / t.tn);
    const uint32_t box[4] = {BK, (uint32_t)t.tw, (uint32_t)t.th, (uint32_t)t.tn};
    if (s2) {
      const uint64_t dims[4] = {(uint64_t)a.K1, (uint64_t)GW, (uint64_t)GH, (uint64_t)a.nimg};
      const uint64_t str[3] = {(uint64_t)a.K1 * 4, (uint64_t)a.K1 * 4 * a.W, (uint64_t)a.K1 * 2 * a.W * a.H};
      if (make_tmap_f16(&p.tmA, a.A, 4, dims, str, box, 1)) return 3;
      for (int k = 1; k < 4; ++k)
        if (make_tmap_f16(&p2.tmP[k - 1], a.A + ((long long)(k >> 1) * a.W + (k & 1)) * a.K1, 4, dims, str, box, 1)) return 3;
    } else {
      const uint64_t dims[4] = {(uint64_t)a.K1, (uint64_t)a.W, (uint64_t)a.H, (uint64_t)a.nimg};
      const uint64_t str[3] = {(uint64_t)a.lda1 * 2, (uint64_t)a.lda1 * 2 * a.W, (uint64_t)a.lda1 * 2 * a.W * a.H};
      if (make_tmap_f16(&p.tmA, a.A, 4, dims, str, box, 1)) return 3;
      const long long shift[3] = {(long long)a.W * a.lda1, (long long)a.lda1, (long long)(a.W + 1) * a.lda1};
      for (int k = 0; k < 3; ++k) {
        const bool used = k == 2 ? ps.sub_short == 3 : ((ps.sub_short >> k) & 1) != 0;
        if (used && make_tmap_f16(&ps.tmS[k], a.A - shift[k], 4, dims, str, box, 1)) return 3;
      }
    }
    if (two) {
      const uint64_t dims[4] = {(uint64_t)a.K2, (uint64_t)a.W, (uint64_t)a.H, (uint64_t)a.nimg};
      const uint64_t str[3] = {(uint64_t)a.lda2 * 2, (uint64_t)a.lda2 * 2 * a.W, (uint64_t)a.lda2 * 2 * a.W * a.H};
      if (make_tmap_f16(&p.tmA2, a.A2, 4, dims, str, box, 1)) return 3;
    }
  } else {
    p.a_rank = 2;
    p.m_tiles = (a.M + BM - 1) / BM;
    const uint32_t box[2] = {BK, BM};
    {
      const uint64_t dims[2] = {(uint64_t)a.K1, (uint64_t)a.M};
      const uint64_t str[1] = {(uint64_t)a.lda1 * 2};
      if (make_tmap_f16(&p.tmA, a.A, 2, dims, str, box, 1)) return 3;
    }
    if (two) {
      const uint64_t dims[2] = {(uint64_t)a.K2, (uint64_t)a.M};
      const uint64_t str[1] = {(uint64_t)a.lda2 * 2};
      if (make_tmap_f16(&p.tmA2, a.A2, 2, dims, str, box, 1)) return 3;
    }
  }

  int bn = a.force_bn;
  if (a.mode == EPI_GEGLU) {
    bn = 2 * kGegluGranule;
    VS_REQUIRE(a.N % bn == 0, "gemm_tc: GEGLU needs N %% %d == 0 (N=%d)", bn, a.N);
    VS_REQUIRE(a.bias != nullptr && a.residual == nullptr && a.rowvec == nullptr, "gemm_tc: GEGLU takes a bias only");
  } else if (bn == 0) {
    bn = pick_bn(p.m_tiles, a.N, p.num_kb);
  }
  VS_REQUIRE(bn == 64 || bn == 128 || bn == 160 || bn == 256, "gemm_tc: unsupported BLOCK_N %d", bn);
  p.n_tiles = (a.N + bn - 1) / bn;
  {
    const uint64_t dims[2] = {(uint64_t)Ktot, (uint64_t)a.N};
    const uint64_t str[1] = {(uint64_t)Ktot * 2};
    const uint32_t box[2] = {BK, (uint32_t)bn};
    if (make_tmap_f16(&p.tmB, a.Bw, 2, dims, str, box, 1)) return 3;
  }
  const int out_cols = (a.mode == EPI_GEGLU) ? a.N / 2 : a.N;
  p.staged = (out_cols % EPI_COLS == 0) && (a.ldc % 8 == 0) && ((reinterpret_cast<uintptr_t>(a.out) & 15) == 0) &&
             (!a.residual || ((a.ldr % 8 == 0) && ((reinterpret_cast<uintptr_t>(a.residual) & 15) == 0))) &&
             (!a.bias || (reinterpret_cast<uintptr_t>(a.bias) & 15) == 0) &&
             (!a.rowvec || ((reinterpret_cast<uintptr_t>(a.rowvec) & 15) == 0 && p.ldrv % 4 == 0));
  if (a.mode == EPI_QUICK_GELU)
    VS_REQUIRE(a.taps == 1 && p.staged && a.residual == nullptr && a.rowvec == nullptr && !a.ln_stats && !a.ln_parts &&
               a.ln_sums_out == nullptr && (bn == 128 || bn == 256),
               "gemm_tc: the quick-GELU epilogue takes a plain GEMM with a bias only, N %% 32 == 0 and BLOCK_N 128 / 256 (got %d)", bn);
  if (!p.staged) VS_REQUIRE(a.mode == EPI_LINEAR, "gemm_tc: GEGLU output needs 32-column aligned, 16-byte strided rows");
  if (a.ln_stats || a.ln_parts) VS_REQUIRE(p.staged && (reinterpret_cast<uintptr_t>(a.ln_u) & 15) == 0, "gemm_tc: folded LayerNorm needs the staged epilogue");
  if (a.ln_sums_out) VS_REQUIRE(p.staged, "gemm_tc: row statistics output needs the staged epilogue (N %% 32 == 0, aligned rows)");
  ProfScope prof(st, a.taps != 1 ? PC_CONV : PC_GEMM, 2.0 * a.M * (double)a.N * Ktot, 1, a.M, a.N, Ktot);
  if (a.mode == EPI_GEGLU) {
    if (const int e = launch_linear_slot<256>(st, p, a); e >= 0) return e;
    if (p.ln_stats || p.ln_parts) return launch<256, EPI_F_GEGLU | EPI_F_LN>(st, p);
    return launch<256, EPI_F_GEGLU>(st, p);
  }
  if (a.mode == EPI_QUICK_GELU) return bn == 256 ? launch<256, EPI_F_QGELU>(st, p) : launch<128, EPI_F_QGELU>(st, p);
  if (s2) {
    VS_REQUIRE(a.residual == nullptr && a.rowvec == nullptr && a.ln_sums_out == nullptr && p.staged,
               "gemm_tc: the stride-2 conv takes a bias only and needs N %% 32 == 0");
    static_cast<GemmParams&>(p2) = p;
    switch (bn) {
      case 64: return launch<64, 0, GemmParamsS2>(st, p2);
      case 128: return launch<128, 0, GemmParamsS2>(st, p2);
      case 256: return launch<256, 0, GemmParamsS2>(st, p2);
      default: return launch<160, 0, GemmParamsS2>(st, p2);
    }
  }
  if (sub && ((OH | OW) & 1)) {
    VS_REQUIRE(a.residual == nullptr && a.rowvec == nullptr && p.staged, "gemm_tc: an odd-sized sub-pixel conv takes a bias only");
    switch (bn) {
      case 64: return launch<64, 0, GemmParamsSub>(st, ps);
      case 128: return launch<128, 0, GemmParamsSub>(st, ps);
      case 256: return launch<256, 0, GemmParamsSub>(st, ps);
      default: return launch<160, 0, GemmParamsSub>(st, ps);
    }
  }
  if (bn == 128 || bn == 160) {
    const int e = bn == 128 ? launch_linear_slot<128>(st, p, a) : launch_linear_slot<160>(st, p, a);
    if (e >= 0) return e;
  }
  switch (bn) {
    case 64: return launch_linear<64>(st, p);
    case 128: return launch_linear<128>(st, p);
    case 256: return launch_linear<256>(st, p);
    default: return launch_linear<160>(st, p);
  }
}

static const __half* subpixel_panel(const __half* w3x3, const __half* wsub, int cout, int cin, int py, int px, bool odd_y,
                                    bool odd_x) {
  const bool ty3 = py == 0 && odd_y, tx3 = px == 0 && odd_x;
  const size_t tap = (size_t)cout * cin;
  if (ty3 && tx3) return w3x3;
  if (ty3) return wsub + (16 + 6 * px) * tap;
  if (tx3) return wsub + (28 + 6 * py) * tap;
  return wsub + (size_t)(2 * py + px) * 4 * tap;
}

int upsample_conv3x3(cudaStream_t st, const __half* x, int nimg, int H, int W, int C, const __half* w3x3, const __half* wsub,
                     const float* bias, int cout, int OH, int OW, __half* out) {
  VS_REQUIRE((OH == 2 * H || OH == 2 * H - 1) && (OW == 2 * W || OW == 2 * W - 1),
             "upsample_conv3x3: output %dx%d is not 2x (or 2x - 1) of the %dx%d input", OH, OW, H, W);
  VS_REQUIRE(w3x3 != nullptr || ((OH & 1) == 0 && (OW & 1) == 0), "upsample_conv3x3: odd output sizes need the 3x3 panel");
  for (int par = 0; par < 4; ++par) {
    GemmArgs g;
    g.A = x; g.K1 = C; g.lda1 = C; g.Bw = subpixel_panel(w3x3, wsub, cout, C, par >> 1, par & 1, OH & 1, OW & 1); g.taps = 4;
    g.sub_py = par >> 1; g.sub_px = par & 1; g.OH = OH; g.OW = OW; g.nimg = nimg; g.H = H; g.W = W; g.M = nimg * H * W;
    g.N = cout; g.bias = bias; g.out = out; g.ldc = cout;
    if (int e = gemm_tc(st, g)) return e;
  }
  return 0;
}

}
```

### videoswap_b200/csrc/kernels.h

```cpp
#pragma once
#include <cuda_fp16.h>
#include <cuda_runtime.h>
#include <stdint.h>

namespace vs {

enum EpiMode { EPI_LINEAR = 0, EPI_GEGLU = 1, EPI_QUICK_GELU = 2 };

struct GemmArgs {
  const __half* A = nullptr;  int K1 = 0;  int lda1 = 0;
  const __half* A2 = nullptr; int K2 = 0;  int lda2 = 0;
  const __half* Bw = nullptr;
  int M = 0, N = 0;
  int taps = 1;
  int sub_py = 0, sub_px = 0;
  int nimg = 0, H = 0, W = 0;
  const float* bias = nullptr;
  const float* rowvec = nullptr;
  int ldrv = 0;
  int pix_per_batch = 1;
  int rv_mod = 0;
  const float* ln_stats = nullptr;
  const float* ln_u = nullptr;
  const float* ln_parts = nullptr;
  int ln_nparts = 0;
  float* ln_sums_out = nullptr;
  const __half* residual = nullptr; int ldr = 0;
  __half* out = nullptr; int ldc = 0;
  int mode = EPI_LINEAR;
  int force_bn = 0;
  int OH = 0, OW = 0;
  int stride2 = 0;
};
int gemm_tc(cudaStream_t st, const GemmArgs& a);
int gemm_n_tiles(const GemmArgs& a);
constexpr int kGegluGranule = 128;

int groupnorm_stats(cudaStream_t st, const __half* x1, int c1, const __half* x2, int c2, int nimg, int hw,
                    int imgs_per_set, int groups, float* sums, bool zero_first = true);
int groupnorm_apply(cudaStream_t st, const __half* x1, int c1, const __half* x2, int c2, int nimg, int hw,
                    int imgs_per_set, int groups, const float* sums, float eps, const float* gamma,
                    const float* beta, bool silu, __half* out, int count_scale = 1);
int groupnorm_frame_fused(cudaStream_t st, const __half* x, int C, int nimg, int hw, int groups, float eps, const float* gamma,
                          const float* beta, bool silu, __half* out);
int layernorm(cudaStream_t st, const __half* x, int rows, int C, const float* gamma, const float* beta,
              const float* pe, int hw, int F, __half* out);

bool ln_fold_supported(int C);
int ln_rowstats(cudaStream_t st, const __half* x, long long rows, int C, float* stats);
int ln_fold(cudaStream_t st, const __half* w, int N, int K, const float* gamma, const float* beta, const float* bias,
            const float* pe, int pe_len, __half* wf, float* u, float* c, float* cpe);

int attention(cudaStream_t st, const __half* q, int ldq, const __half* k, int ldk, const __half* v, int ldv,
              __half* o, int ldo, int batch, int nq, int nk, int heads, int d, long long q_bstride,
              long long kv_bstride, long long o_bstride, int kv_div);
int attention_tc(cudaStream_t st, const __half* q, int ldq, const __half* k, int ldk, const __half* v, int ldv,
                 __half* o, int ldo, int batch, int nq, int nk, int heads, int d, long long q_bstride,
                 long long kv_bstride, long long o_bstride, int kv_div);
int attention_probs(cudaStream_t st, const __half* q, int ldq, const __half* k, int ldk, __half* probs, int batch, int nq, int nk,
                    int heads, int d, long long q_bstride, long long kv_bstride, int kv_div);
int attention_apply_probs(cudaStream_t st, const __half* probs, const __half* v, int ldv, __half* o, int ldo, int batch, int nq,
                          int nk, int heads, int d, long long kv_bstride, long long o_bstride, int kv_div);
int set_option(const char* name, int value);
int get_option(const char* name);
int temporal_attention(cudaStream_t st, const __half* qkv, __half* o, int B, int F, int HW, int C, int heads);
int softmax_rows(cudaStream_t st, __half* s, int rows, int n, int ld, float scale);
int transpose_pad(cudaStream_t st, const __half* src, int rows, int cols, int rows_pad, __half* dst);

int clip_embed(cudaStream_t st, const int* ids, int n, int L, const __half* tok, int vocab, const __half* pos, int C,
               __half* out);
int causal_attention(cudaStream_t st, const __half* qkv, int ldqkv, __half* o, int ldo, int nseq, int L, int heads, int d);

int dift_noise(cudaStream_t st, const __half* moments, const float* eps1, const float* eps2, int n, int E, int h, int w,
               float sf, float sqrt_a, float sqrt_1ma, float* out);
int dift_point_sample(cudaStream_t st, const __half* feat, int n, int E, int h, int w, int C, int H, int W, const int* xy,
                      int P, float* out);
int dift_ensemble_mean(cudaStream_t st, const __half* feat, int n, int E, int h, int w, int C, float* out);
int dift_point_reduce(cudaStream_t st, const float* vecs, int n, int P, int C, const float* src, const int* src_row,
                      float* conf, const uint8_t* accept, float* sums, float* counts, float* means);

int small_linear(cudaStream_t st, const float* x, int rows, int K, const __half* W, const float* bias, int N,
                 bool silu_in, bool silu_out, float* out);
int timestep_embedding(cudaStream_t st, const float* t, int B, int dim, float* out);
int conv_in_3x3(cudaStream_t st, const __half* x, int nimg, int H, int W, int cin, const __half* w, const float* bias,
                int cout, __half* out, __half* scratch = nullptr);
int upsample_nearest2x(cudaStream_t st, const __half* x, int nimg, int H, int W, int C, __half* out, int OH = 0, int OW = 0);
int im2col_s2(cudaStream_t st, const __half* x, int nimg, int H, int W, int C, __half* out);
int add_inplace(cudaStream_t st, __half* x, const __half* r, size_t n, float scale);
int ncfhw_to_nhwc(cudaStream_t st, const void* src, int src_is_f32, int B, int C, int F, int H, int W, __half* dst);
int nhwc_to_ncfhw(cudaStream_t st, const __half* src, int B, int C, int F, int H, int W, void* dst, int dst_is_f32);
int nchw_to_nhwc(cudaStream_t st, const __half* src, int n, int C, int H, int W, float scale, __half* dst);
int vae_latent_in(cudaStream_t st, const void* z, int z_is_f32, int nimg, int h, int w, float divisor, const float* wb, __half* out);
enum ImageFormat { IMG_SAMPLE = 0, IMG_PT = 1, IMG_NP = 2, IMG_PIL = 3 };
int image_postprocess(cudaStream_t st, const __half* x, int nimg, int H, int W, int cs, int format, void* out);
enum VaeImageSource { VAE_IN_U8_NHWC = 0, VAE_IN_F16_NCHW = 1, VAE_IN_F32_NCHW = 2 };
int vae_image_in(cudaStream_t st, const void* x, int src, int nimg, int H, int W, __half* out);
int vae_moments(cudaStream_t st, const __half* x, int nimg, int h, int w, const float* wb, __half* out);
int vae_posterior(cudaStream_t st, const __half* params, const __half* noise, int nimg, int h, int w, float scale, int layout,
                  __half* out);
int cfg_ddim_step(cudaStream_t st, const void* eps2, const void* latents, int is_f32, size_t n, int cfg,
                  float guidance, float a_t, float a_prev, void* out);
int cfg_ddim_step_dev(cudaStream_t st, const void* eps2, const void* latents, int is_f32, size_t n, int cfg,
                      float guidance, const float* d_coef, void* out);
int cfg_ddim_rescale_step(cudaStream_t st, const void* eps2, const void* latents, const void* noise, int is_f32, int S,
                          size_t n_s, int cfg, float guidance, float a_t, float a_prev, float eta, float rescale, void* out);
int cfg_ddim_rescale_step_dev(cudaStream_t st, const void* eps2, const void* latents, const void* noise, int is_f32, int S,
                              size_t n_s, int cfg, float guidance, const float* d_coef, void* out);
int adapter_splat(cudaStream_t st, const float* feat, const float* tracks, const int* point_mask, int F, int P, int C,
                  int h, int w, float rate, int coord_fp16, float scale, __half* maps);

}
struct vs_comm;
namespace vs {
int comm_rank(const vs_comm* c);
int comm_size(const vs_comm* c);
int comm_all_reduce_sum_f32(vs_comm* c, cudaStream_t st, float* buf, size_t n);
int comm_all_gather(vs_comm* c, cudaStream_t st, const void* send, void* recv, size_t bytes);
int comm_all_to_all_rows(vs_comm* c, cudaStream_t st, const __half* src, __half* dst, int n_outer, size_t chunk, int gather);

int blend_mask(cudaStream_t st, const __half* const* maps, const int* map_res, int n_maps, int n_prompts, int frames, int heads,
               int words, const float* alpha, int pool, int h, int w, float threshold, int both, float* mask);
int latent_blend(cudaStream_t st, const void* x_src, void* x_tgt, const float* mask, int is_f32, int channels, int frames, int hw);

int pack_conv3x3(cudaStream_t st, const __half* w, int cout, int cin, __half* out);
int pack_conv_subpixel(cudaStream_t st, const __half* w, int cout, int cin, __half* out, bool odd_panels = false);
int upsample_conv3x3(cudaStream_t st, const __half* x, int nimg, int H, int W, int C, const __half* w3x3, const __half* wsub,
                     const float* bias, int cout, int OH, int OW, __half* out);
int pack_geglu(cudaStream_t st, const __half* w, const __half* b, int hidden, int K, int granule, __half* wout,
               float* bout);
int f16_to_f32(cudaStream_t st, const __half* x, size_t n, float* out);

}
```

### videoswap_b200/ops.py

```python
from __future__ import annotations

import ctypes as C
from typing import Optional, Sequence

import torch

from . import _lib

GEGLU_GRANULE = 128
EPI_LINEAR, EPI_GEGLU, EPI_QUICK_GELU = 0, 1, 2


def set_option(name: str, value: int):
    _lib.call("vs_set_option", name.encode(), int(value))


def _stream() -> int:
    return torch.cuda.current_stream().cuda_stream


def _p(t: Optional[torch.Tensor]):
    return None if t is None else C.c_void_p(t.data_ptr())


def _chk16(*ts):
    for t in ts:
        if t is not None:
            assert t.is_cuda and t.dtype == torch.float16 and t.is_contiguous(), "expected contiguous fp16 CUDA tensor"


def _chk32(*ts):
    for t in ts:
        if t is not None:
            assert t.is_cuda and t.dtype == torch.float32 and t.is_contiguous(), "expected contiguous fp32 CUDA tensor"


def _ptr(t: Optional[torch.Tensor]) -> int:
    return 0 if t is None else t.data_ptr()


def _out16(out, shape, device):
    if out is None:
        return torch.empty(shape, dtype=torch.float16, device=device)
    _chk16(out)
    assert tuple(out.shape) == tuple(shape), f"out has shape {tuple(out.shape)}, expected {tuple(shape)}"
    return out


def _chk_rowvec(rv, N):
    if rv is not None:
        assert rv.is_cuda and rv.dtype == torch.float32 and rv.dim() == 2 and rv.shape[1] == N and rv.stride(1) == 1, \
            "expected an fp32 [rows, N] CUDA row-vector table with unit column stride"


def max_column_tiles(N, force_bn=0):
    bn = force_bn or (64 if N <= 64 else 128)
    return -(-N // bn)


def _gemm_ex(**fields):
    d = _lib.GemmDescStruct()
    d.taps = 1
    d.pix_per_batch = 1
    for k, v in fields.items():
        setattr(d, k, v)
    _lib.call("vs_gemm_ex", _stream(), C.byref(d))


def gemm(A, W, bias=None, residual=None, A2=None, rowvec=None, pix_per_batch=1, mode=EPI_LINEAR, force_bn=0, out=None,
         ln_sums=None):
    _chk16(A, W, residual, A2)
    _chk32(bias, ln_sums)
    M, K1 = A.shape
    K2 = 0 if A2 is None else A2.shape[1]
    N = W.shape[0]
    assert W.shape[1] == K1 + K2
    _chk_rowvec(rowvec, N)
    oc = N // 2 if mode == EPI_GEGLU else N
    out = _out16(out, (M, oc), A.device)
    if ln_sums is not None:
        assert ln_sums.dim() == 3 and ln_sums.shape[1:] == (M, 2) and ln_sums.shape[0] >= max_column_tiles(N, force_bn)
    _gemm_ex(A=_ptr(A), K1=K1, lda1=K1, A2=_ptr(A2), K2=K2, lda2=K2, Bw=_ptr(W), M=M, N=N, bias=_ptr(bias),
             rowvec=_ptr(rowvec), ldrv=0 if rowvec is None else rowvec.stride(0), pix_per_batch=pix_per_batch,
             ln_sums_out=_ptr(ln_sums), residual=_ptr(residual), ldr=oc, out=_ptr(out), ldc=oc, mode=mode, force_bn=force_bn)
    return out


def pack_conv3x3(w):
    _chk16(w)
    co, ci = w.shape[:2]
    out = torch.empty((co, 9 * ci), dtype=torch.float16, device=w.device)
    _lib.call("vs_pack_conv3x3", _stream(), _p(w), co, ci, _p(out))
    return out


def pack_geglu(w, b):
    _chk16(w, b)
    hidden, K = w.shape[0] // 2, w.shape[1]
    wout = torch.empty_like(w)
    bout = torch.empty((2 * hidden,), dtype=torch.float32, device=w.device)
    _lib.call("vs_pack_geglu", _stream(), _p(w), _p(b), hidden, K, _p(wout), _p(bout))
    return wout, bout


def conv3x3(x, w_packed, bias=None, x2=None, rowvec=None, imgs_per_batch=1, residual=None, out=None):
    _chk16(x, w_packed, x2, residual)
    _chk32(bias)
    n, H, W, C1 = x.shape
    C2 = 0 if x2 is None else x2.shape[3]
    co = w_packed.shape[0]
    _chk_rowvec(rowvec, co)
    out = _out16(out, (n, H, W, co), x.device)
    _gemm_ex(A=_ptr(x), K1=C1, lda1=C1, A2=_ptr(x2), K2=C2, lda2=C2, Bw=_ptr(w_packed), M=n * H * W, N=co, taps=9, nimg=n,
             H=H, W=W, bias=_ptr(bias), rowvec=_ptr(rowvec), ldrv=0 if rowvec is None else rowvec.stride(0),
             pix_per_batch=imgs_per_batch * H * W, residual=_ptr(residual), ldr=co, out=_ptr(out), ldc=co)
    return out


def conv3x3_s2(x, w_packed, bias=None):
    _chk16(x, w_packed)
    n, H, W, Ci = x.shape
    co = w_packed.shape[0]
    Ho, Wo = (H - 1) // 2 + 1, (W - 1) // 2 + 1
    scratch = torch.empty((n * Ho * Wo, 9 * Ci), dtype=torch.float16, device=x.device)
    out = torch.empty((n, Ho, Wo, co), dtype=torch.float16, device=x.device)
    _lib.call("vs_conv3x3_s2", _stream(), _p(x), n, H, W, Ci, _p(w_packed), co, _p(bias), _p(scratch), _p(out))
    return out


def upsample_conv3x3(x, w, bias=None):
    _chk16(x, w)
    _chk32(bias)
    n, H, W, Ci = x.shape
    co = w.shape[0]
    wsub = torch.empty((16 * co * Ci,), dtype=torch.float16, device=x.device)
    out = torch.empty((n, 2 * H, 2 * W, co), dtype=torch.float16, device=x.device)
    _lib.call("vs_upsample_conv3x3", _stream(), _p(x), n, H, W, Ci, _p(w), co, _p(bias), _p(wsub), _p(out))
    return out


def pack_conv_subpixel(w):
    _chk16(w)
    co, ci = w.shape[:2]
    out = torch.empty((4, co, 4 * ci), dtype=torch.float16, device=w.device)
    _lib.call("vs_pack_conv_subpixel", _stream(), _p(w), co, ci, _p(out))
    return out


def upsample_conv3x3_packed(x, wsub, bias=None):
    _chk16(x, wsub)
    _chk32(bias)
    n, H, W, Ci = x.shape
    co = wsub.shape[1]
    assert tuple(wsub.shape) == (4, co, 4 * Ci), "expected pack_conv_subpixel panels"
    out = torch.empty((n, 2 * H, 2 * W, co), dtype=torch.float16, device=x.device)
    for par in range(4):
        _gemm_ex(A=_ptr(x), K1=Ci, lda1=Ci, Bw=_ptr(wsub[par]), M=n * H * W, N=co, taps=4, sub_py=par >> 1, sub_px=par & 1,
                 nimg=n, H=H, W=W, bias=_ptr(bias), out=_ptr(out), ldc=co)
    return out


def upsample_conv3x3_sized(x, w, bias, OH, OW, out=None):
    _chk16(x, w, out)
    _chk32(bias)
    n, H, W, Ci = x.shape
    co = w.shape[0]
    panels = torch.empty((49 * co * Ci,), dtype=torch.float16, device=x.device)
    if out is None:
        out = torch.empty((n, OH, OW, co), dtype=torch.float16, device=x.device)
    assert out.is_contiguous() and out.numel() >= n * OH * OW * co
    _lib.call("vs_upsample_conv3x3_sized", _stream(), _p(x), n, H, W, Ci, _p(w), co, _p(bias), OH, OW, _p(panels), _p(out))
    return out


def upsample_nearest(x, OH, OW):
    _chk16(x)
    n, H, W, Cc = x.shape
    out = torch.empty((n, OH, OW, Cc), dtype=torch.float16, device=x.device)
    _lib.call("vs_upsample_nearest", _stream(), _p(x), n, H, W, Cc, OH, OW, _p(out))
    return out


def groupnorm(x1, gamma, beta, groups, eps, imgs_per_set=1, silu=False, x2=None):
    _chk16(x1, x2)
    _chk32(gamma, beta)
    n, H, W, c1 = x1.shape
    c2 = 0 if x2 is None else x2.shape[3]
    sums = torch.empty((n // imgs_per_set, groups, 2), dtype=torch.float32, device=x1.device)
    out = torch.empty((n, H, W, c1 + c2), dtype=torch.float16, device=x1.device)
    _lib.call("vs_groupnorm", _stream(), _p(x1), c1, _p(x2), c2, n, H * W, imgs_per_set, groups, eps, _p(gamma), _p(beta),
              int(silu), _p(sums), _p(out))
    return out


def groupnorm_stats(x1, sums, groups, imgs_per_set, x2=None, zero_first=True):
    _chk16(x1, x2)
    _chk32(sums)
    n, H, W, c1 = x1.shape
    c2 = 0 if x2 is None else x2.shape[3]
    assert tuple(sums.shape) == (n // imgs_per_set, groups, 2)
    _lib.call("vs_groupnorm_stats", _stream(), _p(x1), c1, _p(x2), c2, n, H * W, imgs_per_set, groups, _p(sums),
              int(zero_first))
    return sums


def groupnorm_apply(x1, sums, gamma, beta, groups, eps, imgs_per_set, count_scale=1, silu=False, x2=None):
    _chk16(x1, x2)
    _chk32(sums, gamma, beta)
    n, H, W, c1 = x1.shape
    c2 = 0 if x2 is None else x2.shape[3]
    out = torch.empty((n, H, W, c1 + c2), dtype=torch.float16, device=x1.device)
    _lib.call("vs_groupnorm_apply", _stream(), _p(x1), c1, _p(x2), c2, n, H * W, imgs_per_set, groups, _p(sums), eps,
              _p(gamma), _p(beta), int(silu), int(count_scale), _p(out))
    return out


def layernorm(x, gamma, beta, pe=None, hw=1, F=1):
    _chk16(x)
    _chk32(gamma, beta, pe)
    rows, Cc = x.shape
    out = torch.empty_like(x)
    _lib.call("vs_layernorm", _stream(), _p(x), rows, Cc, _p(gamma), _p(beta), _p(pe), hw, F, _p(out))
    return out


def ln_linear(x, W, gamma, beta, bias=None, pe=None, hw=1, frames=1, mode=EPI_LINEAR):
    _chk16(x, W)
    _chk32(gamma, beta, bias, pe)
    M, Cc = x.shape
    N = W.shape[0]
    dev = x.device
    wf = torch.empty_like(W)
    u = torch.empty((N,), dtype=torch.float32, device=dev)
    c = torch.empty((N,), dtype=torch.float32, device=dev)
    cpe = torch.empty((pe.shape[0], N), dtype=torch.float32, device=dev) if pe is not None else None
    stats = torch.empty((M, 2), dtype=torch.float32, device=dev)
    out = torch.empty((M, N // 2 if mode == EPI_GEGLU else N), dtype=torch.float16, device=dev)
    _lib.call("vs_ln_linear", _stream(), _p(x), M, Cc, _p(W), _p(bias), N, _p(gamma), _p(beta), _p(pe),
              0 if pe is None else pe.shape[0], hw, frames, mode, _p(wf), _p(u), _p(c), _p(cpe), _p(stats), _p(out))
    return out


def linear_ln_linear(x0, W0, b0, W, gamma, beta, residual=None, bias=None, mode=EPI_LINEAR, pe=None, hw=1, frames=1):
    _chk16(x0, W0, W, residual)
    _chk32(b0, gamma, beta, bias, pe)
    M, K0 = x0.shape
    Cc, N = W0.shape[0], W.shape[0]
    dev = x0.device
    x = torch.empty((M, Cc), dtype=torch.float16, device=dev)
    wf = torch.empty_like(W)
    u = torch.empty((N,), dtype=torch.float32, device=dev)
    c = torch.empty((N,), dtype=torch.float32, device=dev)
    cpe = torch.empty((pe.shape[0], N), dtype=torch.float32, device=dev) if pe is not None else None
    cap = 16
    parts = torch.empty((cap, M, 2), dtype=torch.float32, device=dev)
    out = torch.empty((M, N // 2 if mode == EPI_GEGLU else N), dtype=torch.float16, device=dev)
    _lib.call("vs_linear_ln_linear", _stream(), _p(x0), M, K0, _p(W0), _p(b0), _p(residual), Cc, _p(x), _p(W), _p(bias), N,
              _p(gamma), _p(beta), _p(pe), 0 if pe is None else pe.shape[0], hw, frames, mode, _p(wf), _p(u), _p(c), _p(cpe),
              _p(parts), cap, _p(out))
    return x, out


def attention(q, k, v, heads, kv_div=1):
    B, nq, Cc = q.shape
    nk = k.shape[1]
    d = Cc // heads
    for t in (q, k, v):
        assert t.dtype == torch.float16 and t.stride(2) == 1
    out = torch.empty((B, nq, Cc), dtype=torch.float16, device=q.device)
    _lib.call("vs_attention", _stream(), _p(q), q.stride(1), _p(k), k.stride(1), _p(v), v.stride(1), _p(out), Cc, B, nq, nk,
              heads, d, q.stride(0), k.stride(0), nq * Cc, kv_div)
    return out


def attention_probs(q, k, heads, kv_div=1):
    B, nq, Cc = q.shape
    nk = k.shape[1]
    probs = torch.empty((B, heads, nq, nk), dtype=torch.float16, device=q.device)
    _lib.call("vs_attention_probs", _stream(), _p(q), q.stride(1), _p(k), k.stride(1), _p(probs), B, nq, nk, heads, Cc // heads,
              q.stride(0), k.stride(0), kv_div)
    return probs


def attention_apply_probs(probs, v, heads, kv_div=1):
    _chk16(probs)
    B, _, nq, nk = probs.shape
    Cc = v.shape[2]
    out = torch.empty((B, nq, Cc), dtype=torch.float16, device=probs.device)
    _lib.call("vs_attention_apply_probs", _stream(), _p(probs), _p(v), v.stride(1), _p(out), Cc, B, nq, nk, heads, Cc // heads,
              v.stride(0), nq * Cc, kv_div)
    return out


def scores(q, k, out):
    _chk16(q, k, out)
    nq, d = q.shape
    nk = k.shape[0]
    assert k.shape[1] == d and out.dim() == 2 and out.shape[0] == nq and out.shape[1] >= nk
    _gemm_ex(A=_ptr(q), K1=d, lda1=d, Bw=_ptr(k), M=nq, N=nk, out=_ptr(out), ldc=out.shape[1])
    return out


def softmax_rows(s, n, scale):
    _chk16(s)
    rows, ld = s.shape
    _lib.call("vs_softmax_rows", _stream(), _p(s), rows, n, ld, float(scale))
    return s


def transpose_pad(x, rows_pad, out=None):
    _chk16(x)
    rows, cols = x.shape
    out = _out16(out, (cols, rows_pad), x.device)
    _lib.call("vs_transpose_pad", _stream(), _p(x), rows, cols, rows_pad, _p(out))
    return out


def vae_latent_in(z, divisor, wb):
    assert z.is_cuda and z.dtype in (torch.float16, torch.float32) and z.is_contiguous() and z.dim() == 4 and z.shape[1] == 4, \
        "expected contiguous [n, 4, h, w] fp16 / fp32 CUDA latents"
    _chk32(wb)
    assert wb.numel() == 20
    n, _, h, w = z.shape
    out = torch.empty((n, h, w, 4), dtype=torch.float16, device=z.device)
    _lib.call("vs_vae_latent_in", _stream(), _p(z), int(z.dtype == torch.float32), n, h, w, float(divisor), _p(wb), _p(out))
    return out


IMG_SAMPLE, IMG_PT, IMG_NP, IMG_PIL = 0, 1, 2, 3


def image_postprocess(x, fmt):
    _chk16(x)
    n, H, W, Cc = x.shape
    shape = (n, 3, H, W) if fmt in (IMG_SAMPLE, IMG_PT) else (n, H, W, 3)
    dtype = {IMG_SAMPLE: torch.float16, IMG_PT: torch.float32, IMG_NP: torch.float32, IMG_PIL: torch.uint8}[fmt]
    out = torch.empty(shape, dtype=dtype, device=x.device)
    _lib.call("vs_image_postprocess", _stream(), _p(x), n, H, W, Cc, fmt, _p(out))
    return out


def downsample_conv3x3(x, w_packed, bias=None):
    _chk16(x, w_packed)
    _chk32(bias)
    n, H, W, Ci = x.shape
    co = w_packed.shape[0]
    assert w_packed.shape[1] == 9 * Ci, "expected a pack_conv3x3 panel"
    out = torch.empty((n, H // 2, W // 2, co), dtype=torch.float16, device=x.device)
    _lib.call("vs_downsample_conv3x3", _stream(), _p(x), n, H, W, Ci, _p(w_packed), co, _p(bias), _p(out))
    return out


VAE_IN_U8_NHWC, VAE_IN_F16_NCHW, VAE_IN_F32_NCHW = 0, 1, 2


def vae_image_in(x):
    assert x.is_cuda and x.is_contiguous() and x.dim() == 4, "expected a contiguous 4-D CUDA tensor"
    if x.dtype == torch.uint8:
        assert x.shape[3] == 3, "uint8 frames are [n, H, W, 3]"
        src, (n, H, W) = VAE_IN_U8_NHWC, x.shape[:3]
    else:
        assert x.dtype in (torch.float16, torch.float32) and x.shape[1] == 3, "float images are [n, 3, H, W] fp16 / fp32"
        src = VAE_IN_F16_NCHW if x.dtype == torch.float16 else VAE_IN_F32_NCHW
        n, _, H, W = x.shape
    out = torch.empty((n, H, W, 4), dtype=torch.float16, device=x.device)
    _lib.call("vs_vae_image_in", _stream(), _p(x), src, n, H, W, _p(out))
    return out


def vae_moments(x, wb):
    _chk16(x)
    _chk32(wb)
    n, h, w, Cc = x.shape
    assert Cc == 8 and wb.numel() == 72
    out = torch.empty((n, 8, h, w), dtype=torch.float16, device=x.device)
    _lib.call("vs_vae_moments", _stream(), _p(x), n, h, w, _p(wb), _p(out))
    return out


def vae_posterior(params, noise=None, scale=1.0, video=False):
    _chk16(params, noise)
    n, c8, h, w = params.shape
    assert c8 == 8 and (noise is None or tuple(noise.shape) == (n, 4, h, w))
    out = torch.empty((1, 4, n, h, w) if video else (n, 4, h, w), dtype=torch.float16, device=params.device)
    _lib.call("vs_vae_posterior", _stream(), _p(params), _p(noise), n, h, w, float(scale), int(video), _p(out))
    return out


def clip_embed(ids, tok, pos):
    _chk16(tok, pos)
    assert ids.is_cuda and ids.dtype == torch.int32 and ids.is_contiguous() and ids.dim() == 2, "expected int32 [n, L] CUDA ids"
    n, L = ids.shape
    vocab, Cc = tok.shape
    assert pos.shape[1] == Cc and pos.shape[0] >= L
    out = torch.empty((n * L, Cc), dtype=torch.float16, device=tok.device)
    _lib.call("vs_clip_embed", _stream(), _p(ids), n, L, _p(tok), vocab, _p(pos), Cc, _p(out))
    return out


def causal_attention(qkv, nseq, L, heads, out=None):
    assert qkv.is_cuda and qkv.dtype == torch.float16 and qkv.dim() == 2 and qkv.stride(1) == 1 and qkv.shape[0] == nseq * L
    Cc = qkv.shape[1] // 3
    if out is None:
        out = torch.empty((nseq * L, Cc), dtype=torch.float16, device=qkv.device)
    assert out.is_cuda and out.dtype == torch.float16 and out.stride(1) == 1 and tuple(out.shape) == (nseq * L, Cc), \
        "out: fp16 [nseq L, C] CUDA tensor with unit column stride"
    _lib.call("vs_causal_attention", _stream(), _p(qkv), qkv.stride(0), _p(out), out.stride(0), nseq, L, heads, Cc // heads)
    return out


def temporal_attention(qkv, heads):
    _chk16(qkv)
    B, F, HW, C3 = qkv.shape
    out = torch.empty((B, F, HW, C3 // 3), dtype=torch.float16, device=qkv.device)
    _lib.call("vs_temporal_attention", _stream(), _p(qkv), _p(out), B, F, HW, C3 // 3, heads)
    return out


def conv_in(x, w, bias, scratch="alloc"):
    _chk16(x, w)
    _chk32(bias)
    n, H, W, ci = x.shape
    co = w.shape[0]
    if isinstance(scratch, str):
        assert scratch == "alloc"
        scratch = torch.empty(((n * H * W + co) * 64,), dtype=torch.float16, device=x.device) if ci == 4 else None
    _chk16(scratch)
    if scratch is not None:
        assert scratch.numel() >= (n * H * W + co) * 64
    out = torch.empty((n, H, W, co), dtype=torch.float16, device=x.device)
    _lib.call("vs_conv_in", _stream(), _p(x), n, H, W, ci, _p(w), _p(bias), co, _p(scratch), _p(out))
    return out


def upsample2x(x):
    _chk16(x)
    n, H, W, Cc = x.shape
    out = torch.empty((n, 2 * H, 2 * W, Cc), dtype=torch.float16, device=x.device)
    _lib.call("vs_upsample2x", _stream(), _p(x), n, H, W, Cc, _p(out))
    return out


def ddim_coefficients(alpha_t: float, alpha_prev: float, eta: Optional[float] = None):
    import math
    if eta is None:
        c_x = math.sqrt(alpha_prev) / math.sqrt(alpha_t)
        c_e = math.sqrt(1.0 - alpha_prev) - math.sqrt(alpha_prev) * math.sqrt(1.0 - alpha_t) / math.sqrt(alpha_t)
        return c_x, c_e
    if eta < 0:
        raise ValueError(f"eta must be >= 0, got {eta}")
    at, ap = float(alpha_t), float(alpha_prev)
    c_n = 0.0 if eta == 0 else float(eta) * math.sqrt((1.0 - ap) / (1.0 - at) * (1.0 - at / ap))
    c_x = math.sqrt(ap) / math.sqrt(at)
    c_e = math.sqrt(1.0 - ap - c_n * c_n) - math.sqrt(ap) * math.sqrt(1.0 - at) / math.sqrt(at)
    return c_x, c_e, c_n


def cfg_ddim_step(eps2, latents, guidance, alpha_t=None, alpha_prev=None, cfg=True, out=None, coef=None):
    assert eps2.dtype == latents.dtype and eps2.is_contiguous() and latents.is_contiguous()
    is_f32 = int(latents.dtype == torch.float32)
    if out is None:
        out = torch.empty_like(latents)
    if coef is not None:
        _chk32(coef)
        _lib.call("vs_cfg_ddim_step_dev", _stream(), _p(eps2), _p(latents), is_f32, latents.numel(), int(cfg), float(guidance),
                  _p(coef), _p(out))
        return out
    _lib.call("vs_cfg_ddim_step", _stream(), _p(eps2), _p(latents), is_f32, latents.numel(), int(cfg), float(guidance),
              float(alpha_t), float(alpha_prev), _p(out))
    return out


def cfg_ddim_rescale_step(eps2, latents, guidance, alpha_t=None, alpha_prev=None, eta=0.0, guidance_rescale=0.0,
                          noise=None, cfg=True, out=None, coef=None):
    S = latents.shape[0]
    assert eps2.dtype == latents.dtype and eps2.is_contiguous() and latents.is_contiguous()
    assert eps2.numel() == latents.numel() * (2 if cfg else 1), "eps2 must hold (2 if cfg else 1) x latents' elements"
    if noise is not None:
        assert noise.dtype == latents.dtype and noise.is_contiguous() and noise.shape == latents.shape
    is_f32 = int(latents.dtype == torch.float32)
    if out is None:
        out = torch.empty_like(latents)
    n_s = latents.numel() // S
    if coef is not None:
        _chk32(coef)
        assert coef.numel() >= 4
        _lib.call("vs_cfg_ddim_rescale_step_dev", _stream(), _p(eps2), _p(latents), _p(noise), is_f32, S, n_s, int(cfg),
                  float(guidance), _p(coef), _p(out))
        return out
    _lib.call("vs_cfg_ddim_rescale_step", _stream(), _p(eps2), _p(latents), _p(noise), is_f32, S, n_s, int(cfg),
              float(guidance), float(alpha_t), float(alpha_prev), float(eta), float(guidance_rescale), _p(out))
    return out


def adapter_level(w0, b0, w1, b1, point_embedding, tracks, h, w, rate, point_mask=None, coord_fp16=True, scale=1.0):
    _chk16(w0, b0, w1, b1)
    _chk32(point_embedding, tracks)
    mid, E = w0.shape
    Cc = w1.shape[0]
    F, P = tracks.shape[:2]
    ws = torch.empty((mid + Cc + P * (mid + Cc),), dtype=torch.float32, device=w0.device)
    out = torch.empty((F, h, w, Cc), dtype=torch.float16, device=w0.device)
    _lib.call("vs_adapter_level", _stream(), _p(w0), _p(b0), _p(w1), _p(b1), E, mid, Cc, _p(point_embedding), _p(tracks),
              _p(point_mask), F, P, h, w, float(rate), int(coord_fp16), float(scale), _p(ws), _p(out))
    return out


def dift_noise(moments, eps1, eps2, scaling_factor, sqrt_a, sqrt_1ma):
    _chk16(moments)
    _chk32(eps1, eps2)
    n, c8, h, w = moments.shape
    assert c8 == 8 and eps1.shape == eps2.shape and eps1.dim() == 4 and tuple(eps1.shape[1:]) == (4, h, w)
    assert eps1.shape[0] % n == 0, "noise rows must be a whole ensemble per frame"
    E = eps1.shape[0] // n
    out = torch.empty((n * E, 4, 1, h, w), dtype=torch.float32, device=moments.device)
    _lib.call("vs_dift_noise", _stream(), _p(moments), _p(eps1), _p(eps2), n, E, h, w, float(scaling_factor), float(sqrt_a),
              float(sqrt_1ma), _p(out))
    return out


def dift_point_sample(feat, size, xy):
    _chk16(feat)
    assert xy.is_cuda and xy.dtype == torch.int32 and xy.is_contiguous() and xy.dim() == 3 and xy.shape[2] == 2
    n, E, h, w, Cc = feat.shape
    assert xy.shape[0] == n
    P = xy.shape[1]
    out = torch.empty((n, P, Cc), dtype=torch.float32, device=feat.device)
    if P:
        _lib.call("vs_dift_point_sample", _stream(), _p(feat), n, E, h, w, Cc, int(size[0]), int(size[1]), _p(xy), P, _p(out))
    return out


def dift_ensemble_mean(feat):
    _chk16(feat)
    n, E, h, w, Cc = feat.shape
    out = torch.empty((n, Cc, h, w), dtype=torch.float32, device=feat.device)
    _lib.call("vs_dift_ensemble_mean", _stream(), _p(feat), n, E, h, w, Cc, _p(out))
    return out


def dift_point_cosine(vecs, src, src_row):
    _chk32(vecs, src)
    assert src_row.is_cuda and src_row.dtype == torch.int32 and src_row.is_contiguous()
    n, P, Cc = vecs.shape
    assert src.dim() == 2 and src.shape[1] == Cc and tuple(src_row.shape) == (n, P)
    conf = torch.empty((n, P), dtype=torch.float32, device=vecs.device)
    _lib.call("vs_dift_point_reduce", _stream(), _p(vecs), n, P, Cc, _p(src), _p(src_row), _p(conf), None, None, None, None)
    return conf


def dift_point_reduce(vecs, accept):
    _chk32(vecs)
    n, P, Cc = vecs.shape
    acc = accept.to(device=vecs.device, dtype=torch.uint8).contiguous()
    assert tuple(acc.shape) == (n, P)
    sums = torch.empty((P, Cc), dtype=torch.float32, device=vecs.device)
    means = torch.empty_like(sums)
    counts = torch.empty((P,), dtype=torch.float32, device=vecs.device)
    _lib.call("vs_dift_point_reduce", _stream(), _p(vecs), n, P, Cc, None, None, None, _p(acc), _p(sums), _p(counts), _p(means))
    return sums, counts, means
```

Measured before the change: 11.24.

## Add 256-row GEMM tiles for wide 3x3 convs and revise tile cost model

```diff
diff --git a/include/videoswap_b200.h b/include/videoswap_b200.h
--- a/include/videoswap_b200.h
+++ b/include/videoswap_b200.h
@@ -107,8 +107,10 @@
   int force_bn;
   int OH, OW;
   int stride2;
+  int force_bm;
 } vs_gemm_desc;
 int vs_gemm_ex(void* stream, const vs_gemm_desc* desc);
+int vs_gemm_tile(const vs_gemm_desc* desc, int* rows, int* block_n);
 int vs_pack_conv3x3(void* stream, const void* d_w, int cout, int cin, void* d_out);
 int vs_pack_geglu(void* stream, const void* d_w, const void* d_b, int hidden, int K, void* d_wout, float* d_bout);
 int vs_groupnorm(void* stream, const void* d_x1, int c1, const void* d_x2, int c2, int nimg, int hw, int imgs_per_set,
diff --git a/videoswap_b200/_lib.py b/videoswap_b200/_lib.py
--- a/videoswap_b200/_lib.py
+++ b/videoswap_b200/_lib.py
@@ -55,6 +55,7 @@
         ("force_bn", _I),
         ("OH", _I), ("OW", _I),
         ("stride2", _I),
+        ("force_bm", _I),
     ]
 
 _SIGNATURES = {
@@ -93,6 +94,7 @@
     "vs_cfg_ddim_rescale_step_dev": (_I, [_P, _P, _P, _P, _I, _I, _SZ, _I, _F, _P, _P]),
     "vs_adapter_level": (_I, [_P, _P, _P, _P, _P, _I, _I, _I, _P, _P, _P, _I, _I, _I, _I, _F, _I, _F, _P, _P]),
     "vs_gemm_ex": (_I, [_P, C.POINTER(GemmDescStruct)]),
+    "vs_gemm_tile": (_I, [C.POINTER(GemmDescStruct), C.POINTER(_I), C.POINTER(_I)]),
     "vs_pack_conv3x3": (_I, [_P, _P, _I, _I, _P]),
     "vs_pack_geglu": (_I, [_P, _P, _P, _I, _I, _P, _P]),
     "vs_groupnorm": (_I, [_P, _P, _I, _P, _I, _I, _I, _I, _I, _F, _P, _P, _I, _P, _P]),
diff --git a/videoswap_b200/csrc/api.cu b/videoswap_b200/csrc/api.cu
--- a/videoswap_b200/csrc/api.cu
+++ b/videoswap_b200/csrc/api.cu
@@ -58,8 +58,7 @@
   return adapter_splat(st, feat, d_tracks, d_mask, F, P, C, h, w, rate, coord_fp16, scale, (__half*)d_map);
 }
 
-extern "C" int vs_gemm_ex(void* stream, const vs_gemm_desc* d) {
-  VS_REQUIRE(d != nullptr, "vs_gemm_ex: null descriptor");
+static GemmArgs gemm_args(const vs_gemm_desc* d) {
   GemmArgs g;
   g.A = (const __half*)d->A; g.K1 = d->K1; g.lda1 = d->lda1;
   g.A2 = (const __half*)d->A2; g.K2 = d->K2; g.lda2 = d->lda2;
@@ -79,7 +78,18 @@
   g.force_bn = d->force_bn;
   g.OH = d->OH; g.OW = d->OW;
   g.stride2 = d->stride2;
-  return gemm_tc((cudaStream_t)stream, g);
+  g.force_bm = d->force_bm;
+  return g;
+}
+
+extern "C" int vs_gemm_ex(void* stream, const vs_gemm_desc* d) {
+  VS_REQUIRE(d != nullptr, "vs_gemm_ex: null descriptor");
+  return gemm_tc((cudaStream_t)stream, gemm_args(d));
+}
+
+extern "C" int vs_gemm_tile(const vs_gemm_desc* d, int* rows, int* block_n) {
+  VS_REQUIRE(d != nullptr && rows != nullptr && block_n != nullptr, "vs_gemm_tile: null pointer");
+  return gemm_tile(gemm_args(d), rows, block_n);
 }
 
 extern "C" int vs_pack_conv3x3(void* stream, const void* d_w, int cout, int cin, void* d_out) {
diff --git a/videoswap_b200/csrc/gemm.cu b/videoswap_b200/csrc/gemm.cu
--- a/videoswap_b200/csrc/gemm.cu
+++ b/videoswap_b200/csrc/gemm.cu
@@ -10,7 +10,6 @@
 constexpr int BM = 128;
 constexpr int WG_M = 64;
 constexpr int BK = 64;
-constexpr int A_STAGE_BYTES = BM * BK * 2;
 constexpr uint64_t A_HALF_DESC = (WG_M * BK * 2) >> 4;
 constexpr int GEMM_THREADS = 384;
 constexpr int SMEM_LIMIT = 227 * 1024;
@@ -78,10 +77,12 @@
   static constexpr int BYTES = RES ? (END + 1023) / 1024 * 1024 : (END + 127) / 128 * 128;
 };
 
-template <int BN, int SLOT_BYTES = 0>
+template <int BN, int SLOT_BYTES = 0, int TM = BM>
 struct Cfg {
   static constexpr bool COOP = BN > 160;
+  static constexpr bool SHARED = COOP || TM == 256;
   static constexpr int HALVES = COOP ? 1 : 2;
+  static constexpr int A_STAGE_BYTES = TM * BK * 2;
   static constexpr int B_STAGE_BYTES = BN * BK * 2;
   static constexpr int STAGE_BYTES = A_STAGE_BYTES + B_STAGE_BYTES;
   static constexpr int STAGES_RAW = SLOT_BYTES ? (SMEM_LIMIT - 1024 - 256 - EPI_BYTES - 2 * SLOT_BYTES) / STAGE_BYTES
@@ -93,19 +94,20 @@
   static_assert(STAGES >= 3, "pipeline too shallow");
   static_assert(SMEM_BYTES <= SMEM_LIMIT, "shared memory");
   static_assert(BN % 32 == 0 && BN <= 256, "wgmma N");
+  static_assert(TM == 128 || (TM == 256 && !COOP && SLOT_BYTES == 0), "256-row tiles: BN <= 160, no epilogue slots");
 };
 
 __device__ __forceinline__ uint32_t sw64_off(int row, int chunk) {
   return (uint32_t)(row * 64 + ((chunk ^ ((row >> 1) & 3)) << 4));
 }
 
-template <int BN, int EPI, typename Params>
+template <int BN, int EPI, typename Params, int TM = BM>
 __global__ void __launch_bounds__(GEMM_THREADS, 1) gemm_tc_kernel(const __grid_constant__ Params p) {
   constexpr bool SUB = std::is_same<Params, GemmParamsSub>::value;
   constexpr bool S2 = std::is_same<Params, GemmParamsS2>::value;
   constexpr bool SLOT = std::is_same<Params, GemmParamsEpi>::value;
   using ES = EpiSlot<BN, EPI>;
-  using C = Cfg<BN, SLOT ? ES::BYTES : 0>;
+  using C = Cfg<BN, SLOT ? ES::BYTES : 0, TM>;
   static_assert(!SLOT || ((C::COOP == ((EPI & EPI_F_GEGLU) != 0)) && (EPI & EPI_F_QGELU) == 0), "epilogue slots: ping-pong linears and cooperative GEGLUs");
   constexpr bool GEGLU = (EPI & EPI_F_GEGLU) != 0, HAS_RES = (EPI & EPI_F_RES) != 0, HAS_RV = (EPI & EPI_F_RV) != 0;
   constexpr bool LN = (EPI & EPI_F_LN) != 0;
@@ -148,7 +150,7 @@
     }
     for (int s = 0; s < C::STAGES; ++s) {
       mbar_init(full_bar(s), 1);
-      mbar_init(empty_bar(s), C::COOP ? 8 : 4);
+      mbar_init(empty_bar(s), C::SHARED ? 8 : 4);
     }
     fence_barrier_init();
   }
@@ -215,7 +217,7 @@
         i0 = (m_tile / (p.tiles_x * p.tiles_y)) * p.TN;
       }
       const int n0 = n_tile * BN;
-      const int m0 = m_tile * BM;
+      const int m0 = m_tile * TM;
       int kcoord = 0;
       int dy = p.tap_y0, dx = tap_x0;
       int r = 0;
@@ -240,7 +242,7 @@
           mbar_expect_tx(fb, C::STAGE_BYTES);
           if (conv) tma_load_4d(a_dst, tm, fb, c, x0 + ox, y0 + oy, i0);
           else tma_load_2d(a_dst, tm, fb, c, m0);
-          tma_load_2d(a_dst + A_STAGE_BYTES, &p.tmB, fb, kcoord, n0);
+          tma_load_2d(a_dst + C::A_STAGE_BYTES, &p.tmB, fb, kcoord, n0);
         }
         __syncwarp();
         kcoord += BK;
@@ -276,7 +278,7 @@
       }
       return ((img < p.nimg) && (y < p.H) && (x < p.W)) ? (img * p.OH + y * p.osy + p.ooy) * p.OW + x * p.osx + p.oox : -1;
     }
-    const int px = m_tile * BM + row;
+    const int px = m_tile * TM + row;
     return px < p.M ? px : -1;
   };
 
@@ -285,20 +287,20 @@
   uint32_t s = 0, ph = 0;
   for (int t = blockIdx.x, j = 0; t < total_tiles; t += gridDim.x, ++j) {
     const int m_tile = t / p.n_tiles, n_tile = t % p.n_tiles;
-    if (!C::COOP && (j & 1) != g) {
+    if (!C::SHARED && (j & 1) != g) {
       const uint32_t sn = s + (uint32_t)num_kb;
       ph ^= (sn / (uint32_t)nst) & 1u;
       s = sn % (uint32_t)nst;
       continue;
     }
-    if (!C::COOP && j > 0) named_bar_sync(bar_mine, 256);
+    if (!C::SHARED && j > 0) named_bar_sync(bar_mine, 256);
     uint32_t prev = 0;
     for (int kb = 0; kb < num_kb; ++kb) {
       mbar_wait(full_bar(s), ph);
       wgmma_fence();
       const uint32_t a_addr = smem_base + s * C::STAGE_BYTES;
-      const uint64_t da = gmma_desc_sw128(a_addr) + (C::COOP ? (uint64_t)g * A_HALF_DESC : 0);
-      const uint64_t db = gmma_desc_sw128(a_addr + A_STAGE_BYTES);
+      const uint64_t da = gmma_desc_sw128(a_addr) + (C::SHARED ? (uint64_t)(g * C::HALVES) * A_HALF_DESC : 0);
+      const uint64_t db = gmma_desc_sw128(a_addr + C::A_STAGE_BYTES);
 #pragma unroll
       for (int k = 0; k < BK / 16; ++k) {
 #pragma unroll
@@ -313,7 +315,7 @@
       prev = s;
       if (++s == (uint32_t)nst) { s = 0; ph ^= 1; }
     }
-    if (!C::COOP && t + (int)gridDim.x < total_tiles) named_bar_arrive(bar_other, 256);
+    if (!C::SHARED && t + (int)gridDim.x < total_tiles) named_bar_arrive(bar_other, 256);
     wgmma_wait<0>();
     if (lane == 0) mbar_arrive(empty_bar(prev));
     const int js = j & 1;
@@ -323,7 +325,7 @@
     const int n0 = n_tile * BN;
 #pragma unroll
     for (int hh = 0; hh < C::HALVES; ++hh) {
-      const int r0 = WG_M * (C::COOP ? g : hh) + rbase;
+      const int r0 = WG_M * (C::SHARED ? g * C::HALVES + hh : hh) + rbase;
       int pix[2];
       pix[0] = tile_pixel(m_tile, r0);
       pix[1] = tile_pixel(m_tile, r0 + 8);
@@ -508,12 +510,12 @@
 
 struct ConvTile { int tw, th, tn; };
 
-ConvTile pick_conv_tile(int nimg, int H, int W) {
-  ConvTile best{1, 1, BM};
+ConvTile pick_conv_tile(int nimg, int H, int W, int rows) {
+  ConvTile best{1, 1, rows};
   long long best_cost = -1;
-  for (int tw = 1; tw <= BM; tw *= 2) {
-    for (int th = 1; tw * th <= BM; th *= 2) {
-      const int tn = BM / (tw * th);
+  for (int tw = 1; tw <= rows; tw *= 2) {
+    for (int th = 1; tw * th <= rows; th *= 2) {
+      const int tn = rows / (tw * th);
       if (tw > 256 || th > 256 || tn > 256) continue;
       const long long cost = (long long)((W + tw - 1) / tw) * tw * ((H + th - 1) / th) * th * ((nimg + tn - 1) / tn) * tn;
       if (best_cost < 0 || cost < best_cost || (cost == best_cost && tw > best.tw)) {
@@ -525,25 +527,40 @@
   return best;
 }
 
-template <int BN, int EPI, typename Params = GemmParams>
+template <int BN, int EPI, typename Params = GemmParams, int TM = BM>
 int launch(cudaStream_t st, const Params& p) {
-  using C = Cfg<BN, std::is_same<Params, GemmParamsEpi>::value ? EpiSlot<BN, EPI>::BYTES : 0>;
+  using C = Cfg<BN, std::is_same<Params, GemmParamsEpi>::value ? EpiSlot<BN, EPI>::BYTES : 0, TM>;
   static bool configured = false;
   if (!configured) {
-    VS_CHECK_CUDA(cudaFuncSetAttribute(gemm_tc_kernel<BN, EPI, Params>, cudaFuncAttributeMaxDynamicSharedMemorySize, C::SMEM_BYTES));
+    VS_CHECK_CUDA(cudaFuncSetAttribute(gemm_tc_kernel<BN, EPI, Params, TM>, cudaFuncAttributeMaxDynamicSharedMemorySize, C::SMEM_BYTES));
     configured = true;
   }
   const int total = p.m_tiles * p.n_tiles;
   int ctas = num_sms();
   const int cap = get_option("gemm_ctas");
   if (cap > 0 && cap < ctas) ctas = cap;
-  return launch_pdl(gemm_tc_kernel<BN, EPI, Params>, dim3(total < ctas ? total : ctas), dim3(GEMM_THREADS), C::SMEM_BYTES, st, 1, p);
+  return launch_pdl(gemm_tc_kernel<BN, EPI, Params, TM>, dim3(total < ctas ? total : ctas), dim3(GEMM_THREADS), C::SMEM_BYTES, st, 1, p);
+}
+
+int epi_flags(const GemmParams& p) {
+  return (p.residual ? EPI_F_RES : 0) | (p.rowvec ? EPI_F_RV : 0) | ((p.ln_stats || p.ln_parts) ? EPI_F_LN : 0) |
+         (p.ln_sums_out ? EPI_F_LNOUT : 0);
+}
+
+bool rows256_epi(int epi) { return epi == 0 || epi == EPI_F_RV || epi == EPI_F_RES; }
+
+int launch_rows256(cudaStream_t st, const GemmParams& p) {
+  switch (epi_flags(p)) {
+    case 0: return launch<160, 0, GemmParams, 256>(st, p);
+    case EPI_F_RV: return launch<160, EPI_F_RV, GemmParams, 256>(st, p);
+    case EPI_F_RES: return launch<160, EPI_F_RES, GemmParams, 256>(st, p);
+    default: set_error("gemm_tc: no 256-row tile for epilogue combination 0x%x", epi_flags(p)); return 2;
+  }
 }
 
 template <int BN>
 int launch_linear(cudaStream_t st, const GemmParams& p) {
-  const int epi = (p.residual ? EPI_F_RES : 0) | (p.rowvec ? EPI_F_RV : 0) | ((p.ln_stats || p.ln_parts) ? EPI_F_LN : 0) |
-                  (p.ln_sums_out ? EPI_F_LNOUT : 0);
+  const int epi = epi_flags(p);
   switch (epi) {
     case EPI_F_LNOUT: return launch<BN, EPI_F_LNOUT>(st, p);
     case EPI_F_LNOUT | EPI_F_RES: return launch<BN, EPI_F_LNOUT | EPI_F_RES>(st, p);
@@ -596,40 +613,81 @@
   }
 }
 
-int pick_bn(int m_tiles, int N, int num_kb) {
-  if (N <= 64) return 64;
-  int best = 128;
+struct Tile { int bm, bn; };
+
+constexpr int kEpiKb = 3;
+Tile pick_tile(int mt128, int mt256, int N, int num_kb, bool rows256, int force_bm, int force_bn) {
+  if (force_bn == 0 && N <= 64) return Tile{128, 64};
+  Tile best{force_bm == 256 ? 256 : 128, force_bn ? force_bn : 128};
   long long best_cost = -1;
-  const int cand[3] = {128, 160, 256};
-  for (int i = 0; i < 3; ++i) {
-    const int bn = cand[i];
-    if (bn != 128 && N % bn != 0) continue;
-    const long long tiles = (long long)m_tiles * ((N + bn - 1) / bn);
+  const Tile cand[4] = {{128, 128}, {128, 160}, {128, 256}, {256, 160}};
+  for (const Tile& c : cand) {
+    if ((force_bm && c.bm != force_bm) || (force_bn && c.bn != force_bn)) continue;
+    if (c.bm == 256 && !rows256) continue;
+    if (!force_bn && c.bn != 128 && N % c.bn != 0) continue;
+    const long long tiles = (long long)(c.bm == 256 ? mt256 : mt128) * ((N + c.bn - 1) / c.bn);
     const long long waves = (tiles + num_sms() - 1) / num_sms();
-    const long long cost = waves * (16 + bn / 8);
-    if (best_cost < 0 || cost < best_cost || (cost == best_cost && num_kb >= 40)) {
+    const bool shared = c.bm == 256 || c.bn == 256;
+    const long long cost = (c.bm / 8 + c.bn / 8) * (shared ? waves * (num_kb + kEpiKb) : waves * num_kb + kEpiKb);
+    if (best_cost < 0 || cost < best_cost || (cost == best_cost && num_kb >= 40 && c.bm * c.bn > best.bm * best.bn)) {
       best_cost = cost;
-      best = bn;
+      best = c;
     }
   }
   return best;
 }
 
 int ilog2(int v) { int l = 0; while ((1 << l) < v) ++l; return l; }
+
+int m_tiles_of(const GemmArgs& a, int rows) {
+  if (a.taps == 1) return (a.M + rows - 1) / rows;
+  const int GH = a.stride2 ? a.H / 2 : a.H, GW = a.stride2 ? a.W / 2 : a.W;
+  const ConvTile t = pick_conv_tile(a.nimg, GH, GW, rows);
+  return ((GW + t.tw - 1) / t.tw) * ((GH + t.th - 1) / t.th) * ((a.nimg + t.tn - 1) / t.tn);
+}
+
+Tile plan_tile(const GemmArgs& a, int num_kb) {
+  const bool odd_sub = a.taps == 4 && (((a.OH > 0 ? a.OH : 2 * a.H) | (a.OW > 0 ? a.OW : 2 * a.W)) & 1);
+  const int epi = (a.residual ? EPI_F_RES : 0) | (a.rowvec ? EPI_F_RV : 0) | ((a.ln_stats || a.ln_parts) ? EPI_F_LN : 0) |
+                  (a.ln_sums_out ? EPI_F_LNOUT : 0);
+  const bool conv256 = a.mode == EPI_LINEAR && a.taps != 1 && !a.stride2 && !odd_sub && num_kb > 10 && rows256_epi(epi) &&
+                       (a.force_bn == 0 || a.force_bn == 160);
+  const bool rows256 = conv256 && (a.force_bm == 256 || (a.N >= 1280 && a.N % 160 == 0));
+  if (a.force_bm == 256 && !rows256) return Tile{0, 0};
+  if (a.mode == EPI_GEGLU) return Tile{128, 2 * kGegluGranule};
+  return pick_tile(m_tiles_of(a, 128), rows256 ? m_tiles_of(a, 256) : 0, a.N, num_kb, rows256, a.force_bm, a.force_bn);
+}
+
+int num_kb_of(const GemmArgs& a) {
+  const bool two = a.A2 != nullptr && a.K2 > 0;
+  const int kb_tap = (a.K1 + BK - 1) / BK + (two ? a.K2 / BK : 0);
+  if (a.taps == 1 || a.taps == 9) return kb_tap * a.taps;
+  const int OH = a.OH > 0 ? a.OH : 2 * a.H, OW = a.OW > 0 ? a.OW : 2 * a.W;
+  return kb_tap * (a.sub_py == 0 && (OH & 1) ? 3 : 2) * (a.sub_px == 0 && (OW & 1) ? 3 : 2);
+}
 
 }
 
 int gemm_n_tiles(const GemmArgs& a) {
   if (a.taps != 1) return 0;
-  int bn = a.force_bn;
-  if (a.mode == EPI_GEGLU) bn = 2 * kGegluGranule;
-  else if (bn == 0) bn = pick_bn((a.M + BM - 1) / BM, a.N, (a.K1 + BK - 1) / BK + a.K2 / BK);
-  return (a.N + bn - 1) / bn;
+  const int bn = plan_tile(a, num_kb_of(a)).bn;
+  return bn > 0 ? (a.N + bn - 1) / bn : 0;
+}
+
+int gemm_tile(const GemmArgs& a, int* rows, int* bn) {
+  VS_REQUIRE(a.force_bm == 0 || a.force_bm == 128 || a.force_bm == 256, "gemm_tc: force_bm must be 0, 128 or 256 (got %d)", a.force_bm);
+  const Tile t = plan_tile(a, num_kb_of(a));
+  VS_REQUIRE(t.bm != 0, "gemm_tc: no 256-row tile for this launch (3x3 / even sub-pixel conv, K > 640, BLOCK_N 160, bias "
+                        "with at most one of row vector / residual)");
+  *rows = t.bm;
+  *bn = t.bn;
+  return 0;
 }
 
 int gemm_tc(cudaStream_t st, const GemmArgs& a) {
   VS_REQUIRE(a.A && a.Bw && a.out, "gemm_tc: null pointer");
   VS_REQUIRE(a.taps == 1 || a.taps == 9 || a.taps == 4, "gemm_tc: taps must be 1, 9 (3x3) or 4 (sub-pixel)");
+  VS_REQUIRE(a.force_bm == 0 || a.force_bm == 128 || a.force_bm == 256, "gemm_tc: force_bm must be 0, 128 or 256 (got %d)", a.force_bm);
   VS_REQUIRE(a.K1 % 8 == 0 && a.K2 % 8 == 0, "gemm_tc: K must be a multiple of 8 (TMA 16-byte strides)");
   VS_REQUIRE((long long)a.M * (a.ldc > a.ldr ? a.ldc : a.ldr) < (1LL << 40) && a.M < (1 << 30), "gemm_tc: M too large");
   const bool two = a.A2 != nullptr && a.K2 > 0;
@@ -679,6 +737,10 @@
                      !a.ln_stats && !a.ln_parts,
                      "gemm_tc: the stride-2 conv takes one dense NHWC source of even height and width (got %dx%d)", a.H, a.W);
   const int GH = s2 ? a.H / 2 : a.H, GW = s2 ? a.W / 2 : a.W;
+  const Tile tile = plan_tile(a, p.num_kb);
+  VS_REQUIRE(tile.bm != 0, "gemm_tc: no 256-row tile for this launch (3x3 / even sub-pixel conv, K > 640, BLOCK_N 160, bias "
+                           "with at most one of row vector / residual)");
+  const int TMr = tile.bm;
   if (a.taps != 1) {
     VS_REQUIRE(a.nimg > 0 && GH > 0 && GW > 0 && a.M == a.nimg * GH * GW, "gemm_tc: bad conv geometry");
     p.a_rank = 4;
@@ -690,7 +752,7 @@
       ps.sub_short = (sub_ty == 3 ? 1 : 0) | (sub_tx == 3 ? 2 : 0);
       p.osy = p.osx = 2; p.ooy = a.sub_py; p.oox = a.sub_px; p.OH = OH; p.OW = OW;
     }
-    const ConvTile t = pick_conv_tile(a.nimg, GH, GW);
+    const ConvTile t = pick_conv_tile(a.nimg, GH, GW, TMr);
     p.nimg = a.nimg; p.H = GH; p.W = GW; p.TW = t.tw; p.TH = t.th; p.TN = t.tn;
     p.tw_log = ilog2(t.tw);
     p.thw_log = ilog2(t.tw * t.th);
@@ -721,8 +783,8 @@
     }
   } else {
     p.a_rank = 2;
-    p.m_tiles = (a.M + BM - 1) / BM;
-    const uint32_t box[2] = {BK, BM};
+    p.m_tiles = (a.M + TMr - 1) / TMr;
+    const uint32_t box[2] = {BK, (uint32_t)TMr};
     {
       const uint64_t dims[2] = {(uint64_t)a.K1, (uint64_t)a.M};
       const uint64_t str[1] = {(uint64_t)a.lda1 * 2};
@@ -735,13 +797,10 @@
     }
   }
 
-  int bn = a.force_bn;
+  const int bn = tile.bn;
   if (a.mode == EPI_GEGLU) {
-    bn = 2 * kGegluGranule;
     VS_REQUIRE(a.N % bn == 0, "gemm_tc: GEGLU needs N %% %d == 0 (N=%d)", bn, a.N);
     VS_REQUIRE(a.bias != nullptr && a.residual == nullptr && a.rowvec == nullptr, "gemm_tc: GEGLU takes a bias only");
-  } else if (bn == 0) {
-    bn = pick_bn(p.m_tiles, a.N, p.num_kb);
   }
   VS_REQUIRE(bn == 64 || bn == 128 || bn == 160 || bn == 256, "gemm_tc: unsupported BLOCK_N %d", bn);
   p.n_tiles = (a.N + bn - 1) / bn;
@@ -790,6 +849,7 @@
       default: return launch<160, 0, GemmParamsSub>(st, ps);
     }
   }
+  if (TMr == 256) return launch_rows256(st, p);
   if (bn == 128 || bn == 160) {
     const int e = bn == 128 ? launch_linear_slot<128>(st, p, a) : launch_linear_slot<160>(st, p, a);
     if (e >= 0) return e;
diff --git a/videoswap_b200/csrc/kernels.h b/videoswap_b200/csrc/kernels.h
--- a/videoswap_b200/csrc/kernels.h
+++ b/videoswap_b200/csrc/kernels.h
@@ -29,11 +29,13 @@
   __half* out = nullptr; int ldc = 0;
   int mode = EPI_LINEAR;
   int force_bn = 0;
+  int force_bm = 0;
   int OH = 0, OW = 0;
   int stride2 = 0;
 };
 int gemm_tc(cudaStream_t st, const GemmArgs& a);
 int gemm_n_tiles(const GemmArgs& a);
+int gemm_tile(const GemmArgs& a, int* rows, int* bn);
 constexpr int kGegluGranule = 128;
 
 int groupnorm_stats(cudaStream_t st, const __half* x1, int c1, const __half* x2, int c2, int nimg, int hw,
diff --git a/videoswap_b200/ops.py b/videoswap_b200/ops.py
--- a/videoswap_b200/ops.py
+++ b/videoswap_b200/ops.py
@@ -58,17 +58,27 @@
     return -(-N // bn)
 
 
-def _gemm_ex(**fields):
+def _gemm_desc(fields):
     d = _lib.GemmDescStruct()
     d.taps = 1
     d.pix_per_batch = 1
     for k, v in fields.items():
         setattr(d, k, v)
-    _lib.call("vs_gemm_ex", _stream(), C.byref(d))
+    return d
+
+
+def _gemm_ex(**fields):
+    _lib.call("vs_gemm_ex", _stream(), C.byref(_gemm_desc(fields)))
+
+
+def gemm_tile(**fields):
+    rows, bn = C.c_int(0), C.c_int(0)
+    _lib.call("vs_gemm_tile", C.byref(_gemm_desc(fields)), C.byref(rows), C.byref(bn))
+    return rows.value, bn.value
 
 
 def gemm(A, W, bias=None, residual=None, A2=None, rowvec=None, pix_per_batch=1, mode=EPI_LINEAR, force_bn=0, out=None,
-         ln_sums=None):
+         ln_sums=None, force_bm=0):
     _chk16(A, W, residual, A2)
     _chk32(bias, ln_sums)
     M, K1 = A.shape
@@ -82,7 +92,8 @@
         assert ln_sums.dim() == 3 and ln_sums.shape[1:] == (M, 2) and ln_sums.shape[0] >= max_column_tiles(N, force_bn)
     _gemm_ex(A=_ptr(A), K1=K1, lda1=K1, A2=_ptr(A2), K2=K2, lda2=K2, Bw=_ptr(W), M=M, N=N, bias=_ptr(bias),
              rowvec=_ptr(rowvec), ldrv=0 if rowvec is None else rowvec.stride(0), pix_per_batch=pix_per_batch,
-             ln_sums_out=_ptr(ln_sums), residual=_ptr(residual), ldr=oc, out=_ptr(out), ldc=oc, mode=mode, force_bn=force_bn)
+             ln_sums_out=_ptr(ln_sums), residual=_ptr(residual), ldr=oc, out=_ptr(out), ldc=oc, mode=mode, force_bn=force_bn,
+             force_bm=force_bm)
     return out
 
 
```

Result: faster. 11.38, median of 6 (+1.2%).
